# VideoVerses/VideoTuna-dev

Measured on AMD Instinct MI355X. Metric: finetune samples/sec, CogVideoX-2B T2V LoRA 49x480x720 bf16, higher is better.
Workload: dtype bf16; 1 GPU; CogVideoX-2B T2V LoRA finetune 49x480x720 (configs[1]): latents [4,13,16,60,90], text [4,226,4096], r=4 LoRA on to_q/k/v/out, 4 samples per optimizer step as in the YAML (batch_size 2 x accumulate_grad_batches 2), run as 1 micro-batch(es) of 4; mode=lora, model=CogVideoX-2B, micro_batch=4, accumulate_grad_batches=1, global_batch=4, seq_len=17776, layers=30, parallelism=dp1, recompute=none (107 GB of block activations kept in HBM), weights=seeded random init (no checkpoints offline), text=pre-encoded prompt embeddings (synthetic), latents=pre-encoded latents (synthetic)

## Files before the change

include/vt355.h:

```cpp
#ifndef VT355_H
#define VT355_H
#ifdef __cplusplus
extern "C" {
#endif

#define VT_OK 0
#define VT_ERR_BAD_SHAPE (-1)
#define VT_ERR_BAD_ALIGN (-2)
#define VT_ERR_LAUNCH (-3)
#define VT_ERR_UNSUPPORTED (-4)

int vt_version(void);
const char* vt_arch(void);
const char* vt_error_string(int code);

#define VT_EPI_BIAS 0
#define VT_EPI_BIAS_GELU 1
#define VT_EPI_GATED_RES 2
#define VT_EPI_DGELU 3

int vt_gemm_bf16(const void* A, int lda, const void* W, int ldw, void* C, int ldc,
                 int M, int N, int K, const void* bias, int epilogue, int out_fp32,
                 const void* R, int ldr, int r_mod,
                 const float* gate_txt, const float* gate_vid, int gate_bstride, int S, int St,
                 void* C2, int ldc2, const void* U, int ldu, void* stream);
int vt_gemm_set_tile(int mode);
int vt_gemm_bf16_kernel(int M, int N, int K);
int vt_conv_set_tile(int mode);

int vt_gemm_nt_bf16(const void* A, int lda, const void* B, int ldb, float* C, int ldc, int M, int P, int Q,
                    float alpha, int accumulate, void* stream);
int vt_gemm_nt_bf16_unpad(const void* A, int lda, const void* B, int ldb, float* C, int ldc, int M, int P, int Q,
                          float alpha, int accumulate, int row_group, int row_keep, int col_group, int col_keep, void* stream);

int vt_group_colsum(const void* X, int ldx, const void* Y, int ldy, const float* mean, const float* rstd,
                    float* out1, float* out2, long long M, int D, int S, int St, int grouped,
                    long long o_bstride, long long o_segstride, void* stream);

int vt_qk_ln_param_grads(const float* dq_hat, int lddq, const void* dk_hat, int lddk, const void* qkv, int ld,
                         const float* mean, const float* rstd, float* out_2x2x64, long long M, int H,
                         const float* rope_cos, const float* rope_sin, int S, int St, void* stream);
int vt_ln_param_combine(const float* G1, const float* G2, int G, int D, const void* gamma, const void* beta,
                        const float* scale_txt, const float* scale_vid, int bstride, float* dgamma, float* dbeta,
                        float* dshift_txt, float* dshift_vid, float* dscale_txt, float* dscale_vid, int dbstride,
                        int grouped, void* stream);
int vt_small_linear_bwd(const float* dy, int ldy, const void* x, int ldx, const void* W, float* dW, float* db,
                        float* dx, int lddx, int Bn, int N, int K, void* stream);
int vt_silu_bwd(const float* dy, const void* x, float* dx, long long n, void* stream);

int vt_attn_fwd_hd64(const void* q, const void* k, const void* v, void* o, float* lse2,
                     int B, int H, int S,
                     long long q_rs, long long k_rs, long long v_rs, long long o_rs,
                     long long q_bs, long long k_bs, long long v_bs, long long o_bs,
                     float softmax_scale, int q_prescaled, void* stream);

int vt_attn_fwd_bias_hd64(const void* q, const void* k, const void* v, const float* bias_t, void* o, float* lse2,
                          int B, int H, int S,
                          long long q_rs, long long k_rs, long long v_rs, long long o_rs,
                          long long q_bs, long long k_bs, long long v_bs, long long o_bs,
                          float softmax_scale, void* stream);
int vt_gemm_splitk_f32(const void* A, int lda, const void* W, int ldw, float* C, int ldc, int M, int N, int K, int splits, void* stream);
int vt_residual_cast_bf16(const float* acc, long long lda, const void* R, long long ldr, void* out, long long ldo, long long M, int N,
                          void* stream);
long long vt_groupnorm_ws_bytes(int N, int C);
int vt_groupnorm_silu_cl(const void* x, long long ldx, const void* gamma, const void* beta, void* y, long long ldy,
                         int N, long long P, int C, int G, float eps, int silu, float* ws, long long ws_bytes, void* stream);
int vt_causal_conv3d_cl(const void* x, long long ldx, const void* wk, const void* bias, const void* res, long long ldr,
                        void* y, long long ldy, int N, int T, int H, int W, int Cin, int Cout, void* stream);
int vt_downsample_conv2d_cl(const void* x, long long ldx, const void* wk, const void* bias, void* y, long long ldy,
                            int N, int T, int H, int W, int Cin, int Cout, void* stream);
int vt_causal_conv3d_in8_cl(const void* x, const void* wk, const void* bias, void* y, long long ldy,
                            int N, int T, int H, int W, int Cout, void* stream);
int vt_temporal_pool_cl(const void* x, long long ldx, void* y, long long ldy, int N, int T, long long HW, int C, int keep_first,
                        void* stream);
int vt_rmsnorm_bf16(const void* x, long long ldx, const void* w, void* y, long long ldy, long long M, int D, float eps,
                    void* stream);
int vt_gated_gelu_bf16(const void* u, long long ldu, void* y, long long ldy, long long M, int F, void* stream);

int vt_attn_bwd_hd64(const void* q, const void* k, const void* v, const void* o, const void* dout,
                     const float* lse2, float* delta_ws, float* dq_f32, void* dk, void* dv,
                     int B, int H, int S,
                     long long q_rs, long long k_rs, long long v_rs, long long o_rs, long long do_rs,
                     long long dq_rs, long long dk_rs, long long dv_rs,
                     long long q_bs, long long k_bs, long long v_bs, long long o_bs, long long do_bs,
                     long long dq_bs, long long dk_bs, long long dv_bs,
                     float softmax_scale, int q_prescaled, void* chain_ws, long long chain_ws_bytes, void* stream);
long long vt_attn_bwd_chain_ws_bytes(int B, int H, int S);
int vt_attn_bwd_set_chain(int chain_len, int slots);

int vt_ln_modulate_fwd(const void* x, int ldx, void* y, int ldy, const void* gamma, const void* beta,
                       const float* shift_txt, const float* scale_txt, const float* shift_vid,
                       const float* scale_vid, int mod_bstride, float* mean, float* rstd,
                       int M, int D, int S, int St, float eps, void* stream);
int vt_ln_modulate_bwd(const void* dy, int lddy, const void* x, int ldx, const float* mean, const float* rstd,
                       const void* gamma, const float* scale_txt, const float* scale_vid, int mod_bstride,
                       const void* dres, int lddres, void* dx, int lddx,
                       int M, int D, int S, int St, void* stream);

int vt_qk_layernorm_fwd(const void* qkv, int ld, void* out, int ldo, const void* gq, const void* bq,
                        const void* gk, const void* bk, float* mean, float* rstd,
                        long long M, int H, float eps, float q_scale,
                        const float* rope_cos, const float* rope_sin, int S, int St, void* stream);
int vt_qk_layernorm_bwd(const float* dq_hat, int lddq, const void* dk_hat, int lddk, const void* qkv, int ld,
                        const float* mean, const float* rstd, const void* gq, const void* gk,
                        void* dqkv, int ldd, long long M, int H,
                        const float* rope_cos, const float* rope_sin, int S, int St, void* stream);

int vt_gate_mul(const void* x, int ldx, void* y, int ldy, const float* g_txt, const float* g_vid, int bstride,
                long long M, int D, int S, int St, void* stream);
int vt_silu_bf16(const void* x, void* y, long long n, void* stream);
int vt_cast_f32_bf16(const float* x, void* y, long long n, void* stream);
int vt_timestep_embedding(const long long* t, void* out, int B, int D, int flip_sin_to_cos, float freq_shift,
                          void* stream);
int vt_patchify(const void* img, void* tok, int B, int F, int C, int H, int W, int P, int ldt, void* stream);
int vt_unpatchify(const void* tok, void* img, int B, int F, int C, int H, int W, int P, int ldt, void* stream);

int vt_add_noise(const float* x0, const float* noise, const float* sqrt_ab, const float* sqrt_1mab, void* noisy,
                 long long per_sample, int B, void* stream);
int vt_diffusion_loss(const void* vpred, const void* noisy, const float* x0, const float* sqrt_ab,
                      const float* sqrt_1mab, const float* weights, float* loss, float* partials_ws,
                      void* dvpred, long long per_sample, int B, float grad_scale, void* stream);

int vt_diffusion_loss_bwd(const void* vpred, const void* noisy, const float* x0, const float* sqrt_ab,
                          const float* sqrt_1mab, const float* weights, const float* grad_out, void* dvpred,
                          long long per_sample, int B, void* stream);

int vt_adamw(float* p, const float* g, float* m, float* v, void* p_bf16, long long n, float lr, float beta1,
             float beta2, float eps, float weight_decay, int step, float grad_scale, const int* guard, void* stream);

int vt_grad_sqnorm_partials(void);
int vt_grad_sqnorm(const float* g, long long n, float* partials, int slot, void* stream);
int vt_clip_finalize(const float* partials, int nslots, float grad_scale, float max_norm, float* record, void* stream);
int vt_adamw_clip(float* p, const float* g, float* m, float* v, void* p_bf16, long long n, float lr, float beta1,
                  float beta2, float eps, float weight_decay, int step, float grad_scale, const int* guard,
                  const float* clip_coef_dev, float clip_value, void* stream);

int vt_lora_down(const void* X, int ldx, const void* A, int lda, int R, void* T, int ldt, long long M, int K,
                 int zero_cols, void* stream);
int vt_skinny_tn(const void* Big, int ldb, const void* Small, int lds_, int R, float* out, long long osp,
                 long long osr, float alpha, long long M, int P, float* workspace, void* stream);
long long vt_skinny_tn_workspace_bytes(int P);
int vt_lora_up_add(void* dX, int ldx, const void* dT, int ldt, const void* A, int lda, int R, long long M, int K,
                   void* stream);
int vt_lora_pack_b(const float* Bcat, void* Wext, int ldw, int n_adapters, int d_out, int r, float scale, void* stream);
int vt_lora_pack_bt(const float* Bcat, void* WText, int ldwt, int n_adapters, int d_out, int r, float scale, void* stream);

int vt_lora_down_wide(const void* X, int ldx, const void* A, int lda, int n_adapters, int r, int rp, int ext, void* T, int ldt,
                      long long M, int K, void* stream);
int vt_lora_tn_wide(const void* Big, int ldb, const void* Small, int lds_, int R, float* out, long long osp, long long osr,
                    float alpha, long long M, int P, void* stream);
int vt_lora_up_add_wide(void* dX, int ldx, const void* dT, int ldt, const void* A, int lda, int n_adapters, int r, int rp,
                        long long M, int K, void* stream);
int vt_lora_pack_b_wide(const float* Bcat, void* Wext, int ldw, int n_adapters, int d_out, int r, int rp, int ext, float scale,
                        void* stream);
int vt_lora_pack_bt_wide(const float* Bcat, void* WText, int ldwt, int n_adapters, int d_out, int r, int rp, int ext, float scale,
                         void* stream);

int vt_lora_down_drop(const void* X, int ldx, const void* A, int lda, int R, int n_adapters, void* T, int ldt, long long M, int K,
                      int zero_cols, float p, unsigned long long seed, int site0, void* stream);
int vt_skinny_tn_drop(const void* Big, int ldb, const void* Small, int lds_, int R, int n_adapters, float* out, long long osp,
                      long long osr, float alpha, long long M, int P, float* workspace, float p, unsigned long long seed, int site0,
                      void* stream);
int vt_lora_up_add_drop(void* dX, int ldx, const void* dT, int ldt, const void* A, int lda, int R, int n_adapters, long long M, int K,
                        float p, unsigned long long seed, int site0, void* stream);
int vt_lora_down_wide_drop_fits(int n_adapters, int rp);
int vt_lora_down_wide_drop(const void* X, int ldx, const void* A, int lda, int n_adapters, int r, int rp, int ext, void* T, int ldt,
                           long long M, int K, float p, unsigned long long seed, int site0, void* stream);
int vt_lora_tn_wide_drop(const void* Big, int ldb, const void* Small, int lds_, int R, float* out, long long osp, long long osr,
                         float alpha, long long M, int P, float p, unsigned long long seed, int site, void* stream);
int vt_lora_up_add_wide_drop(void* dX, int ldx, const void* dT, int ldt, const void* A, int lda, int n_adapters, int r, int rp,
                             long long M, int K, float p, unsigned long long seed, int site0, void* stream);


int vt_conv_cl(const void* x, long long ldx, const void* wk, const void* bias, const float* sbias, int sbias_ld,
               const void* res, long long ldr, void* y, long long ldy,
               int N, int T, int H, int W, int Cin, int Cout, int KT, int KH, int KW, int pt, int ph, int pw, int stride, void* stream);
int vt_conv_dw_cl(const void* dy, long long lddy, const void* x, long long ldx, float* dw,
                  int N, int T, int H, int W, int Cin, int Cout, int KT, int KH, int KW, int pt, int ph, int pw, int stride,
                  int accumulate, void* stream);
int vt_conv_dw_bias_cl(const void* dy, long long lddy, const void* x, long long ldx, float* dw, float* dbias,
                       int N, int T, int H, int W, int Cin, int Cout, int KT, int KH, int KW, int pt, int ph, int pw, int stride,
                       int accumulate, void* stream);
int vt_transpose_bf16(const void* src, long long src_ld, long long src_boff, void* dst, long long dst_ld, long long dst_boff, int rows, int cols,
                      int nb, void* stream);
int vt_transpose_multi_bf16(const void* table, int njobs, long long total_blocks, void* stream);
int vt_conv_desc_extents(long long ldx, long long lddy, int N, int T, int H, int W, int Cin, int Cout, int KH, int KW, int ph, int pw,
                         int stride, long long* fwd_x_bytes, long long* dw_x_bytes, long long* dw_dy_bytes);
int vt_groupnorm_silu_bwd_cl(const void* dy, long long lddy, const void* x, long long ldx, const void* gamma,
                             const float* ws_fwd, float* ws_bwd, long long ws_bytes, void* dx, long long lddx,
                             float* dgamma, float* dbeta, int N, long long P, int C, int G, int silu, int accumulate, void* stream);
int vt_geglu_fwd(const void* h, long long ldh, void* y, long long ldy, long long M, int F, void* stream);
int vt_geglu_bwd(const void* dy, long long lddy, const void* h, long long ldh, void* dh, long long lddh, long long M, int F, void* stream);
int vt_add_rows_bf16(const void* a, long long lda, const void* b, long long ldb, void* out, long long ldo, long long M, int C, void* stream);
int vt_dropout_bf16(const void* x, long long ldx, void* y, long long ldy, long long M, int C, float p, unsigned long long seed,
                    unsigned long long offset, void* mask_out, void* stream);
int vt_row_map_bf16(const void* src, long long lds, void* out, long long ldo, int mode, long long nb, int d1, int d2, int C,
                    int accumulate, void* stream);
int vt_q_sample(const float* x0, const float* noise, const float* sqrt_ab, const float* sqrt_1mab, const float* scale, void* xt,
                long long per_sample, int B, void* stream);
int vt_mse_loss(const void* pred, const float* target, float* loss, void* dpred, long long total, float grad_scale, void* stream);

int vt_attn_small_fwd(const void* q, const void* k, const void* v, void* o, float* lse2, int NB, int H, int Sq, int Sk,
                      long long q_rs, long long q_bs, long long k_rs, long long k_bs, long long v_rs, long long v_bs,
                      long long o_rs, long long o_bs, float softmax_scale, int mask_block, void* stream);
int vt_attn_small_bwd(const void* q, const void* k, const void* v, const void* o, const void* dout, const float* lse2,
                      void* dq, void* dk, void* dv, float* dk32, float* dv32, int NB, int H, int Sq, int Sk,
                      long long q_rs, long long q_bs, long long k_rs, long long k_bs, long long v_rs, long long v_bs,
                      long long o_rs, long long o_bs, long long do_rs, long long do_bs, long long dq_rs, long long dq_bs,
                      long long dk_rs, long long dv_rs, float softmax_scale, int mask_block, void* stream);

long long vt_attn_dual_ws_floats(int B, int H, int Sq, int rows_per_frame, int Sa, int Sb);
int vt_attn_dual_fwd(const void* q, const void* k, const void* v, const void* k_ip, const void* v_ip, void* o, float* lse2,
                     int B, int H, int Sq, int rows_per_frame, int Sa, int Sb,
                     long long q_rs, long long q_bs, long long k_rs, long long k_bs, long long v_rs, long long v_bs,
                     long long kip_rs, long long kip_bs, long long vip_rs, long long vip_bs, long long o_rs, long long o_bs,
                     float softmax_scale, float img_scale, void* stream);
int vt_attn_dual_bwd(const void* q, const void* k, const void* v, const void* k_ip, const void* v_ip, const void* dout,
                     const float* lse2, void* dq, float* dk32, float* dv32, float* dkip32, float* dvip32, float* ws,
                     long long ws_floats, int B, int H, int Sq, int rows_per_frame, int Sa, int Sb,
                     long long q_rs, long long q_bs, long long k_rs, long long k_bs, long long v_rs, long long v_bs,
                     long long kip_rs, long long kip_bs, long long vip_rs, long long vip_bs, long long do_rs, long long do_bs,
                     long long dq_rs, long long dq_bs, float softmax_scale, float img_scale, void* stream);

int vt_attn_gen_fwd(const void* q, const void* k, const void* v, void* o, float* lse2, const int* kv_len, int head_dim, int hstride,
                    int NB, int H, int Sq, int Sk, long long q_rs, long long q_bs, long long k_rs, long long k_bs, long long v_rs,
                    long long v_bs, long long o_rs, long long o_bs, float softmax_scale, int mask_block, void* stream);
int vt_attn_gen_bwd(const void* q, const void* k, const void* v, const void* o, const void* dout, const float* lse2, const int* kv_len,
                    void* dq, void* dk, void* dv, float* dk32, float* dv32, int head_dim, int hstride, int NB, int H, int Sq, int Sk,
                    long long q_rs, long long q_bs, long long k_rs, long long k_bs, long long v_rs, long long v_bs,
                    long long o_rs, long long o_bs, long long do_rs, long long do_bs, long long dq_rs, long long dq_bs,
                    long long dk_rs, long long dv_rs, float softmax_scale, int mask_block, void* stream);

int vt_opensora_loss(const float* out, const float* x0, const float* noise, const double* coef, double* loss3, float* dout,
                     long long per_channel, int C, int B, float grad_scale, void* stream);

int vt_gemm_fp8(const void* A, int lda, const void* W, int ldw, void* C, int ldc, int M, int N, int K, const void* bias,
                const float* scale_a, const float* scale_w, void* stream);
int vt_quantize_fp8(const void* x, long long ldx, void* y, long long ldy, long long M, int K, float* scale, unsigned int* ws,
                    int given_scale, void* stream);

int vt_gemm_mxfp8(const void* A, int lda, const void* W, int ldw, void* C, int ldc, int M, int N, int K, const void* bias,
                  const float* scale_a, const float* scale_w, int epilogue, const void* residual, int ldr,
                  const float* gate_txt, const float* gate_vid, int gate_bstride, int S, int St, void* pre_act_out, int ldc2,
                  const void* At, int ldat, const void* Wt, int ldwt, int Kt, void* Cq, int ldcq, const float* scale_out,
                  unsigned int* amax, void* stream);
int vt_cast_fp8_scaled(const void* x, long long ldx, void* y, long long ldy, void* cp, long long ldcp, long long M, int K, int L,
                       int Lj, int off, const float* scale, unsigned int* amax, void* stream);
int vt_ln_modulate_fwd_fp8(const void* x, int ldx, void* y, int ldy, const void* gamma, const void* beta,
                           const float* shift_txt, const float* scale_txt, const float* shift_vid,
                           const float* scale_vid, int mod_bstride, float* mean, float* rstd,
// ... 34 lines not shown
```

videotuna-dev_amd/_lib.py:

```python
import ctypes as C
import os

_HERE = os.path.dirname(os.path.abspath(__file__))
_LIB = None


class VtError(RuntimeError):
    pass


def lib_path() -> str:
    return os.environ.get("VT355_LIB") or os.path.join(_HERE, "libvt355.so")


_vp, _i, _ll, _f, _fp = C.c_void_p, C.c_int, C.c_longlong, C.c_float, C.c_void_p
PROTOTYPES = {
    "vt_version": [],
    "vt_arch": [],
    "vt_error_string": [_i],
    "vt_gemm_bf16": [_vp, _i, _vp, _i, _vp, _i, _i, _i, _i, _vp, _i, _i, _vp, _i, _i, _fp, _fp, _i, _i, _i,
                     _vp, _i, _vp, _i, _vp],
    "vt_gemm_set_tile": [_i],
    "vt_gemm_bf16_kernel": [_i, _i, _i],
    "vt_conv_set_tile": [_i],
    "vt_transpose_bf16": [_vp, _ll, _ll, _vp, _ll, _ll, _i, _i, _i, _vp],
    "vt_transpose_multi_bf16": [_vp, _i, _ll, _vp],
    "vt_gemm_nt_bf16": [_vp, _i, _vp, _i, _fp, _i, _i, _i, _i, _f, _i, _vp],
    "vt_gemm_nt_bf16_unpad": [_vp, _i, _vp, _i, _fp, _i, _i, _i, _i, _f, _i, _i, _i, _i, _i, _vp],
    "vt_group_colsum": [_vp, _i, _vp, _i, _fp, _fp, _fp, _fp, _ll, _i, _i, _i, _i, _ll, _ll, _vp],
    "vt_qk_ln_param_grads": [_fp, _i, _vp, _i, _vp, _i, _fp, _fp, _fp, _ll, _i, _fp, _fp, _i, _i, _vp],
    "vt_ln_param_combine": [_fp, _fp, _i, _i, _vp, _vp, _fp, _fp, _i, _fp, _fp, _fp, _fp, _fp, _fp, _i, _i, _vp],
    "vt_small_linear_bwd": [_fp, _i, _vp, _i, _vp, _fp, _fp, _fp, _i, _i, _i, _i, _vp],
    "vt_silu_bwd": [_fp, _vp, _fp, _ll, _vp],
    "vt_attn_fwd_hd64": [_vp, _vp, _vp, _vp, _fp, _i, _i, _i, _ll, _ll, _ll, _ll, _ll, _ll, _ll, _ll, _f, _i, _vp],
    "vt_attn_fwd_bias_hd64": [_vp, _vp, _vp, _fp, _vp, _fp, _i, _i, _i, _ll, _ll, _ll, _ll, _ll, _ll, _ll, _ll, _f, _vp],
    "vt_gemm_splitk_f32": [_vp, _i, _vp, _i, _fp, _i, _i, _i, _i, _i, _vp],
    "vt_residual_cast_bf16": [_fp, _ll, _vp, _ll, _vp, _ll, _ll, _i, _vp],
    "vt_groupnorm_ws_bytes": [_i, _i],
    "vt_groupnorm_silu_cl": [_vp, _ll, _vp, _vp, _vp, _ll, _i, _ll, _i, _i, _f, _i, _fp, _ll, _vp],
    "vt_causal_conv3d_cl": [_vp, _ll, _vp, _vp, _vp, _ll, _vp, _ll, _i, _i, _i, _i, _i, _i, _vp],
    "vt_causal_conv3d_in8_cl": [_vp, _vp, _vp, _vp, _ll, _i, _i, _i, _i, _i, _vp],
    "vt_downsample_conv2d_cl": [_vp, _ll, _vp, _vp, _vp, _ll, _i, _i, _i, _i, _i, _i, _vp],
    "vt_temporal_pool_cl": [_vp, _ll, _vp, _ll, _i, _i, _ll, _i, _i, _vp],
    "vt_rmsnorm_bf16": [_vp, _ll, _vp, _vp, _ll, _ll, _i, _f, _vp],
    "vt_gated_gelu_bf16": [_vp, _ll, _vp, _ll, _ll, _i, _vp],
    "vt_attn_bwd_hd64": [_vp, _vp, _vp, _vp, _vp, _fp, _fp, _fp, _vp, _vp, _i, _i, _i,
                         _ll, _ll, _ll, _ll, _ll, _ll, _ll, _ll, _ll, _ll, _ll, _ll, _ll, _ll, _ll, _ll, _f, _i, _vp, _ll, _vp],
    "vt_attn_bwd_chain_ws_bytes": [_i, _i, _i],
    "vt_attn_bwd_set_chain": [_i, _i],
    "vt_ln_modulate_fwd": [_vp, _i, _vp, _i, _vp, _vp, _fp, _fp, _fp, _fp, _i, _fp, _fp, _i, _i, _i, _i, _f, _vp],
    "vt_ln_modulate_bwd": [_vp, _i, _vp, _i, _fp, _fp, _vp, _fp, _fp, _i, _vp, _i, _vp, _i, _i, _i, _i, _i, _vp],
    "vt_qk_layernorm_fwd": [_vp, _i, _vp, _i, _vp, _vp, _vp, _vp, _fp, _fp, _ll, _i, _f, _f, _fp, _fp, _i, _i, _vp],
    "vt_qk_layernorm_bwd": [_fp, _i, _vp, _i, _vp, _i, _fp, _fp, _vp, _vp, _vp, _i, _ll, _i, _fp, _fp, _i, _i, _vp],
    "vt_gate_mul": [_vp, _i, _vp, _i, _fp, _fp, _i, _ll, _i, _i, _i, _vp],
    "vt_silu_bf16": [_vp, _vp, _ll, _vp],
    "vt_cast_f32_bf16": [_fp, _vp, _ll, _vp],
    "vt_timestep_embedding": [_vp, _vp, _i, _i, _i, _f, _vp],
    "vt_patchify": [_vp, _vp, _i, _i, _i, _i, _i, _i, _i, _vp],
    "vt_unpatchify": [_vp, _vp, _i, _i, _i, _i, _i, _i, _i, _vp],
    "vt_add_noise": [_fp, _fp, _fp, _fp, _vp, _ll, _i, _vp],
    "vt_diffusion_loss": [_vp, _vp, _fp, _fp, _fp, _fp, _fp, _fp, _vp, _ll, _i, _f, _vp],
    "vt_diffusion_loss_bwd": [_vp, _vp, _fp, _fp, _fp, _fp, _fp, _vp, _ll, _i, _vp],
    "vt_adamw": [_fp, _fp, _fp, _fp, _vp, _ll, _f, _f, _f, _f, _f, _i, _f, _vp, _vp],
    "vt_grad_sqnorm_partials": [],
    "vt_grad_sqnorm": [_fp, _ll, _fp, _i, _vp],
    "vt_clip_finalize": [_fp, _i, _f, _f, _fp, _vp],
    "vt_adamw_clip": [_fp, _fp, _fp, _fp, _vp, _ll, _f, _f, _f, _f, _f, _i, _f, _vp, _fp, _f, _vp],
    "vt_lora_down": [_vp, _i, _vp, _i, _i, _vp, _i, _ll, _i, _i, _vp],
    "vt_skinny_tn": [_vp, _i, _vp, _i, _i, _fp, _ll, _ll, _f, _ll, _i, _fp, _vp],
    "vt_skinny_tn_workspace_bytes": [_i],
    "vt_lora_up_add": [_vp, _i, _vp, _i, _vp, _i, _i, _ll, _i, _vp],
    "vt_lora_pack_b": [_fp, _vp, _i, _i, _i, _i, _f, _vp],
    "vt_lora_pack_bt": [_fp, _vp, _i, _i, _i, _i, _f, _vp],
    "vt_lora_down_wide": [_vp, _i, _vp, _i, _i, _i, _i, _i, _vp, _i, _ll, _i, _vp],
    "vt_lora_tn_wide": [_vp, _i, _vp, _i, _i, _fp, _ll, _ll, _f, _ll, _i, _vp],
    "vt_lora_up_add_wide": [_vp, _i, _vp, _i, _vp, _i, _i, _i, _i, _ll, _i, _vp],
    "vt_lora_pack_b_wide": [_fp, _vp, _i, _i, _i, _i, _i, _i, _f, _vp],
    "vt_lora_pack_bt_wide": [_fp, _vp, _i, _i, _i, _i, _i, _i, _f, _vp],
    "vt_lora_down_drop": [_vp, _i, _vp, _i, _i, _i, _vp, _i, _ll, _i, _i, _f, C.c_ulonglong, _i, _vp],
    "vt_skinny_tn_drop": [_vp, _i, _vp, _i, _i, _i, _fp, _ll, _ll, _f, _ll, _i, _fp, _f, C.c_ulonglong, _i, _vp],
    "vt_lora_up_add_drop": [_vp, _i, _vp, _i, _vp, _i, _i, _i, _ll, _i, _f, C.c_ulonglong, _i, _vp],
    "vt_lora_down_wide_drop_fits": [_i, _i],
    "vt_lora_down_wide_drop": [_vp, _i, _vp, _i, _i, _i, _i, _i, _vp, _i, _ll, _i, _f, C.c_ulonglong, _i, _vp],
    "vt_lora_tn_wide_drop": [_vp, _i, _vp, _i, _i, _fp, _ll, _ll, _f, _ll, _i, _f, C.c_ulonglong, _i, _vp],
    "vt_lora_up_add_wide_drop": [_vp, _i, _vp, _i, _vp, _i, _i, _i, _i, _ll, _i, _f, C.c_ulonglong, _i, _vp],
    "vt_conv_cl": [_vp, _ll, _vp, _vp, _fp, _i, _vp, _ll, _vp, _ll] + [_i] * 13 + [_vp],
    "vt_conv_dw_cl": [_vp, _ll, _vp, _ll, _fp] + [_i] * 13 + [_i, _vp],
    "vt_conv_dw_bias_cl": [_vp, _ll, _vp, _ll, _fp, _fp] + [_i] * 13 + [_i, _vp],
    "vt_conv_desc_extents": [_ll, _ll] + [_i] * 11 + [C.POINTER(C.c_longlong)] * 3,
    "vt_groupnorm_silu_bwd_cl": [_vp, _ll, _vp, _ll, _vp, _fp, _fp, _ll, _vp, _ll, _fp, _fp, _i, _ll, _i, _i, _i, _i, _vp],
    "vt_geglu_fwd": [_vp, _ll, _vp, _ll, _ll, _i, _vp],
    "vt_geglu_bwd": [_vp, _ll, _vp, _ll, _vp, _ll, _ll, _i, _vp],
    "vt_add_rows_bf16": [_vp, _ll, _vp, _ll, _vp, _ll, _ll, _i, _vp],
    "vt_dropout_bf16": [_vp, _ll, _vp, _ll, _ll, _i, _f, C.c_ulonglong, C.c_ulonglong, _vp, _vp],
    "vt_row_map_bf16": [_vp, _ll, _vp, _ll, _i, _ll, _i, _i, _i, _i, _vp],
    "vt_q_sample": [_fp, _fp, _fp, _fp, _fp, _vp, _ll, _i, _vp],
    "vt_mse_loss": [_vp, _fp, _fp, _vp, _ll, _f, _vp],
    "vt_attn_small_fwd": [_vp, _vp, _vp, _vp, _fp, _i, _i, _i, _i] + [_ll] * 8 + [_f, _i, _vp],
    "vt_qk_rmsnorm_rope128_fwd": [_vp, _ll, _vp, _ll, _vp, _vp, _fp, _fp, _fp, _ll, _i, _i, _i, _i, _i, _f, _vp],
    "vt_qk_rmsnorm_rope128_bwd": [_vp, _ll, _vp, _ll, _vp, _ll, _vp, _vp, _fp, _fp, _fp, _fp, _fp, _ll, _i, _i, _i, _i, _i, _vp],
    "vt_attn128_fwd": [_vp, _vp, _vp, _vp, _fp, _vp, _i, _i, _i] + [_ll] * 8 + [_f, _vp],
    "vt_attn128_bwd": [_vp, _vp, _vp, _vp, _vp, _fp, _vp, _fp, _fp, _vp, _vp, _vp, _i, _i, _i] + [_ll] * 18 + [_f, _vp],
    "vt_gemm_fp8": [_vp, _i, _vp, _i, _vp, _i, _i, _i, _i, _vp, _fp, _fp, _vp],
    "vt_quantize_fp8": [_vp, _ll, _vp, _ll, _ll, _i, _fp, _vp, _i, _vp],
    "vt_gemm_mxfp8": [_vp, _i, _vp, _i, _vp, _i, _i, _i, _i, _vp, _fp, _fp, _i, _vp, _i, _fp, _fp, _i, _i, _i, _vp, _i,
                      _vp, _i, _vp, _i, _i, _vp, _i, _fp, _vp, _vp],
    "vt_cast_fp8_scaled": [_vp, _ll, _vp, _ll, _vp, _ll, _ll, _i, _i, _i, _i, _fp, _vp, _vp],
    "vt_ln_modulate_fwd_fp8": [_vp, _i, _vp, _i, _vp, _vp, _fp, _fp, _fp, _fp, _i, _fp, _fp, _i, _i, _i, _i, _f, _vp, _i, _fp, _vp, _vp],
    "vt_fp8_scale_update": [_vp, _fp, _fp, _i, _i, _vp],
    "vt_gemm_mxfp8_dx": [_vp, _i, _i, _vp, _i, _vp, _i, _i, _i, _i, _fp, _fp, _i, _vp, _i, _vp, _i, _vp, _i, _vp, _i, _i,
                         _vp, _i, _i, _fp, _vp, _vp],
    "vt_cast_fp8_fmt": [_vp, _ll, _vp, _ll, _vp, _ll, _ll, _i, _i, _i, _i, _i, _fp, _vp, _vp],
    "vt_gate_mul_fp8": [_vp, _i, _vp, _i, _fp, _fp, _i, _ll, _i, _i, _i, _vp, _i, _i, _fp, _vp, _vp],
    "vt_fp8_scale_update_fmax": [_vp, _fp, _fp, _i, _i, _f, _vp],
    "vt_opensora_loss": [_fp, _fp, _fp, _vp, _vp, _fp, _ll, _i, _i, _f, _vp],
    "vt_attn_gen_fwd": [_vp, _vp, _vp, _vp, _fp, _vp, _i, _i, _i, _i, _i, _i] + [_ll] * 8 + [_f, _i, _vp],
    "vt_attn_gen_bwd": [_vp, _vp, _vp, _vp, _vp, _fp, _vp, _vp, _vp, _vp, _fp, _fp, _i, _i, _i, _i, _i, _i] + [_ll] * 14 + [_f, _i, _vp],
    "vt_attn_small_bwd": [_vp, _vp, _vp, _vp, _vp, _fp, _vp, _vp, _vp, _fp, _fp, _i, _i, _i, _i] + [_ll] * 14 + [_f, _i, _vp],
    "vt_attn_dual_ws_floats": [_i] * 6,
    "vt_attn_dual_fwd": [_vp] * 6 + [_fp] + [_i] * 6 + [_ll] * 12 + [_f, _f, _vp],
    "vt_attn_dual_bwd": [_vp] * 6 + [_fp, _vp] + [_fp] * 5 + [_ll] + [_i] * 6 + [_ll] * 14 + [_f, _f, _vp],
}
_RESTYPE = {"vt_arch": C.c_char_p, "vt_error_string": C.c_char_p, "vt_skinny_tn_workspace_bytes": C.c_longlong,
             "vt_attn_bwd_chain_ws_bytes": C.c_longlong, "vt_groupnorm_ws_bytes": C.c_longlong,
             "vt_attn_dual_ws_floats": C.c_longlong}


def load_library():
    global _LIB
    if _LIB is not None:
        return _LIB
    import torch
    path = lib_path()
    if not os.path.exists(path):
        raise VtError(f"{path} not found: build it with `python -c 'import __graft_entry__ as g; g.build()'` "
                      f"(videotuna-dev_amd/csrc/build.sh). There is no CPU / eager fallback.")
    lib = C.CDLL(path)
    for name, args in PROTOTYPES.items():
        fn = getattr(lib, name)
        fn.argtypes = args
        fn.restype = _RESTYPE.get(name, C.c_int)
    _LIB = lib
    return lib


def check(code: int, what: str):
    if code != 0:
        lib = load_library()
        raise VtError(f"{what} failed: {lib.vt_error_string(code).decode()} (code {code})")
```

videotuna-dev_amd/csrc/attn_bwd.hip:

```cpp
#include "common.h"
#include <cstdlib>

#ifndef VT_SUFFIX
#define VT_SUFFIX
#endif
#ifndef VT_PIPE
#define VT_PIPE 1
#endif
#ifndef VT_DRAIN
#define VT_DRAIN 0
#endif
#ifndef VT_DQSHIFT
#define VT_DQSHIFT 0
#endif
#ifndef VT_STATMFMA
#define VT_STATMFMA 0
#endif
#ifndef VT_W8
#define VT_W8 1
#endif
#define BWD_THREADS (VT_W8 ? 512 : 256)
#ifndef VT_DQ16
#define VT_DQ16 0
#endif
#ifndef VT_CHAIN
#define VT_CHAIN 1
#endif
#ifndef VT_ATOM_AUX
#define VT_ATOM_AUX 0
#endif
#ifndef VT_DQPRIO
#define VT_DQPRIO 0
#endif
#ifndef VT_ABL
#define VT_ABL 0
#endif
#ifndef VT_PF
#define VT_PF 1
#endif
#define FENCE() __builtin_amdgcn_sched_barrier(0)
#ifndef DQ_RING
#define DQ_RING 2
#endif
#ifndef VT_DQ2
#define VT_DQ2 0
#endif
#ifndef VT_DMA
#define VT_DMA (VT_PF && VT_W8 && !VT_DQ16)
#endif
#ifndef VT_M16
#define VT_M16 (VT_DMA && !VT_STAMP && !VT_STATMFMA && !PF_R0 && !VT_DMA_LATE && !VT_ABL)
#endif
#ifndef VT_DS4
#define VT_DS4 (VT_M16 && !VT_DQM16)
#endif
#ifndef VT_DQM16
#define VT_DQM16 0
#endif
#ifndef VT_DMA_LATE
#define VT_DMA_LATE 0
#endif
#ifndef PF_TRN
#define PF_TRN 4
#endif
#ifndef PF_ROWN
#define PF_ROWN 2
#endif
#ifndef PF_R0
#define PF_R0 0
#endif
#ifndef VT_STAMP
#define VT_STAMP 0
#endif
#ifndef VT_CLK
#define VT_CLK 0
#endif
#define VT_CAT_(a, b) a##b
#define VT_CAT(a, b) VT_CAT_(a, b)
#define BWD_KERNEL VT_CAT(attn_bwd_hd64_kernel, VT_SUFFIX)
#define BWD_BODY VT_CAT(attn_bwd_body, VT_SUFFIX)
#define DELTA_KERNEL VT_CAT(attn_bwd_delta_kernel, VT_SUFFIX)
#define BWD_ENTRY VT_CAT(vt_attn_bwd_hd64, VT_SUFFIX)

struct AttnBwdParams {
    const bf16_t* q;
    const bf16_t* k;
    const bf16_t* v;
    const bf16_t* dout;
    const float* lse2;
    const float* delta;
    float* dq;
    bf16_t* dk;
    bf16_t* dv;
    int S, H, B;
    long long q_rs, k_rs, v_rs, do_rs, dq_rs, dk_rs, dv_rs;
    long long q_bs, k_bs, v_bs, do_bs, dq_bs, dk_bs, dv_bs;
    float scale, scale_log2;
    int chain_len;
    int* chain_ctr;
    int* chain_flags;
    int* chain_xcc;
    float* chain_tiles;
};

#define KIMG 0
#define DSIMG 32768
#define QTILE 98304
#define LSEOFF 131072
#define STATF 132096
#ifndef BWD_LDS_PAD
#define BWD_LDS_PAD 0
#endif
#define BWD_LDS (132096 + (VT_STATMFMA ? 8192 : (VT_STAMP ? 1024 : BWD_LDS_PAD)))
#if VT_STAMP
#ifndef STAMP_SLOT
#define STAMP_SLOT 40
#endif
#define STAMP_STEP 150
__device__ unsigned VT_CAT(vt_bwd_stamps, VT_SUFFIX)[256];
#define STAMP(i, dep) do { if (rec) { unsigned long long t_; asm volatile("s_memtime %0\n\ts_waitcnt lgkmcnt(0)" : "=s"(t_), "+v"(dep) :: "memory"); \
                                      if (lane == 0) ((unsigned*)(smem + 132096))[w * 16 + (i)] = (unsigned)t_; } } while (0)
#else
#define STAMP(i, dep)
#endif
#define CH_STAGE_BYTES 16384
#ifndef CH_R
#define CH_R 4
#endif
#ifndef CH_HYST
#define CH_HYST 1
#endif
#ifndef CH_SPIN_LIMIT
#define CH_SPIN_LIMIT (1 << 19)
#endif
#define CH_AUX 17

typedef __attribute__((ext_vector_type(8))) short short8v;
typedef int i32x4w __attribute__((ext_vector_type(4)));

__device__ __forceinline__ int swz_f(int row) {
    return (((row >> 1) & 1) << 2) | (((row >> 3) & 1) << 1) | ((row >> 2) & 1);
}
__device__ __forceinline__ int swz4(int row) { return (((row >> 1) & 1) << 3) | (((row >> 3) & 1) << 2) | (((row >> 2) & 1) << 1) | (row & 1); }
__device__ __forceinline__ int swz_off(int row, int chunk) { return row * 128 + ((chunk ^ swz_f(row)) << 4); }

__device__ __forceinline__ bf16x8 tr_pair(const char* p0, const char* p1) {
    short4v lo = __builtin_amdgcn_ds_read_tr16_b64_v4i16((short4v __attribute__((address_space(3)))*)(p0));
    short4v hi = __builtin_amdgcn_ds_read_tr16_b64_v4i16((short4v __attribute__((address_space(3)))*)(p1));
    short8v v8 = {lo[0], lo[1], lo[2], lo[3], hi[0], hi[1], hi[2], hi[3]};
    return __builtin_bit_cast(bf16x8, v8);
}

#if VT_W8
template <bool RAGGED, bool PRESCALED, int ROLE>
__device__ __forceinline__ void BWD_BODY(const AttnBwdParams& p, char* smem, char* stage, const int id, const int slot,
                                         const int cons_end, const int base, const bool l2_prev, const bool l2_next,
                                         bool& dead) {
    constexpr bool has_prod = (ROLE & 1) != 0, has_cons = (ROLE & 2) != 0;
    const int tid = threadIdx.x, lane = tid & 63;
    const int w = __builtin_amdgcn_readfirstlane(tid >> 6);
    const int r = lane & 31, h = lane >> 5, g = lane >> 4, ql = (lane & 15) >> 2, pl = lane & 3;
    const int nkb = (p.S + 255) / 256;
    const int kblk = id % nkb, bh = id / nkb;
    const int head = bh % p.H, b = bh / p.H;
    const int key0 = kblk * 256;

    const bf16_t* qb = p.q + (size_t)b * p.q_bs + head * 64;
    const bf16_t* kb_ = p.k + (size_t)b * p.k_bs + head * 64;
    const bf16_t* vb = p.v + (size_t)b * p.v_bs + head * 64;
    const bf16_t* dob = p.dout + (size_t)b * p.do_bs + head * 64;
    __amdgpu_buffer_rsrc_t rq = make_rsrc(qb, (unsigned)((long long)(p.S - 1) * p.q_rs * 2 + 128));
    __amdgpu_buffer_rsrc_t rk = make_rsrc(kb_, (unsigned)((long long)(p.S - 1) * p.k_rs * 2 + 128));
    __amdgpu_buffer_rsrc_t rv = make_rsrc(vb, (unsigned)((long long)(p.S - 1) * p.v_rs * 2 + 128));
    __amdgpu_buffer_rsrc_t rdo = make_rsrc(dob, (unsigned)((long long)(p.S - 1) * p.do_rs * 2 + 128));
    __amdgpu_buffer_rsrc_t rdq = make_rsrc(p.dq + (size_t)b * p.dq_bs + head * 64, (unsigned)((long long)(p.S - 1) * p.dq_rs * 4 + 256));
    const float* lse_b = p.lse2 + (size_t)bh * p.S;
    const float* dl_b = p.delta + (size_t)bh * p.S;

#pragma unroll
    for (int j = 0; j < 4; ++j) {
        const int i = tid + 512 * j;
        const int key = i >> 3, c = i & 7;
        u32x4 v = __builtin_bit_cast(u32x4, __builtin_amdgcn_raw_buffer_load_b128(rk, (int)((key0 + key) * p.k_rs * 2) + c * 16, 0, 0));
        *(u32x4*)(smem + KIMG + swz_off(key, c)) = v;
    }
#if VT_M16
    const int c15 = lane & 15;
    bf16x8 kf16[2][2], vf16[2][2];
    float kmask16[2];
#pragma unroll
    for (int kt = 0; kt < 2; ++kt) {
        const int key = key0 + 32 * w + 16 * kt + c15;
#pragma unroll
        for (int s = 0; s < 2; ++s) {
            kf16[kt][s] = __builtin_bit_cast(bf16x8, __builtin_amdgcn_raw_buffer_load_b128(rk, (int)(key * p.k_rs * 2) + (32 * s + 8 * g) * 2, 0, 0));
            vf16[kt][s] = __builtin_bit_cast(bf16x8, __builtin_amdgcn_raw_buffer_load_b128(rv, (int)(key * p.v_rs * 2) + (32 * s + 8 * g) * 2, 0, 0));
        }
        kmask16[kt] = (RAGGED && key >= p.S) ? -1.0e30f : 0.f;
    }
#else
    bf16x8 kf[4], vf[4];
    {
        const int key = key0 + 32 * w + r;
#pragma unroll
        for (int s = 0; s < 4; ++s) {
            kf[s] = __builtin_bit_cast(bf16x8, __builtin_amdgcn_raw_buffer_load_b128(rk, (int)(key * p.k_rs * 2) + (16 * s + 8 * h) * 2, 0, 0));
            vf[s] = __builtin_bit_cast(bf16x8, __builtin_amdgcn_raw_buffer_load_b128(rv, (int)(key * p.v_rs * 2) + (16 * s + 8 * h) * 2, 0, 0));
        }
    }
    const float kmask = (RAGGED && (key0 + 32 * w + r) >= p.S) ? -1.0e30f : 0.f;
#endif

#if VT_M16
    int rowrd16[2];
#pragma unroll
    for (int s_ = 0; s_ < 2; ++s_) rowrd16[s_] = c15 * 128 + (((4 * s_ + g) ^ (c15 & 6)) << 4);
    int trA16[4];
#pragma unroll
    for (int dt = 0; dt < 4; ++dt) trA16[dt] = (4 * g + ql) * 128 + (((2 * dt + (pl >> 1)) ^ ((4 * g + ql) & 6)) << 4) + (pl & 1) * 8;
#else
    int rowrd[4];
#pragma unroll
    for (int s = 0; s < 4; ++s) rowrd[s] = r * 128 + (((2 * s + h) ^ swz_f(r)) << 4);
    int trA[2][2];
#pragma unroll
    for (int dt = 0; dt < 2; ++dt)
#pragma unroll
        for (int sec = 0; sec < 2; ++sec) {
            const int fx = ((ql >> 1) << 2) | (sec << 1) | h;
            trA[dt][sec] = (4 * h + ql + 8 * sec) * 128 + (((4 * dt + 2 * (g & 1) + (pl >> 1)) ^ fx) << 4) + (pl & 1) * 8;
        }
#endif
#if VT_DQ16
    const int qt = w >> 1, dh = w & 1;
    int trq16[2], trk16[2][2];
// ... 1330 lines not shown
            for (int i = 0; i < 16; ++i) asm volatile("" ::"v"(dq_acc[i]));
#else
#pragma unroll
            for (int i = 0; i < 16; ++i)
                __builtin_amdgcn_raw_ptr_buffer_atomic_fadd_f32(dq_acc[i] * p.scale, rdq, dq_voff,
                                                                soff + ((i & 3) + 8 * (i >> 2)) * dq_rowb, 0);
#endif
        }
    }
#endif
    const float dk_mul = PRESCALED ? 0.6931471805599453f : p.scale;
#pragma unroll
    for (int kb = 0; kb < 2; ++kb) {
        const int key = key0 + 64 * w + 32 * kb + r;
        if (key < p.S) {
            bf16_t* dkp = p.dk + (size_t)b * p.dk_bs + (size_t)key * p.dk_rs + head * 64;
            bf16_t* dvp = p.dv + (size_t)b * p.dv_bs + (size_t)key * p.dv_rs + head * 64;
#pragma unroll
            for (int dt = 0; dt < 2; ++dt)
#pragma unroll
                for (int gg = 0; gg < 4; ++gg) {
                    u32x2 a, c;
                    a[0] = pack2(dk_acc[kb][dt][4 * gg + 0] * dk_mul, dk_acc[kb][dt][4 * gg + 1] * dk_mul);
                    a[1] = pack2(dk_acc[kb][dt][4 * gg + 2] * dk_mul, dk_acc[kb][dt][4 * gg + 3] * dk_mul);
                    c[0] = pack2(dv_acc[kb][dt][4 * gg + 0], dv_acc[kb][dt][4 * gg + 1]);
                    c[1] = pack2(dv_acc[kb][dt][4 * gg + 2], dv_acc[kb][dt][4 * gg + 3]);
                    *(u32x2*)(dkp + 32 * dt + 8 * gg + 4 * h) = a;
                    *(u32x2*)(dvp + 32 * dt + 8 * gg + 4 * h) = c;
                }
        }
    }
}

#endif

#if VT_CLK
__device__ unsigned VT_CAT(vt_bwd_clk, VT_SUFFIX)[4];
extern "C" int VT_CAT(vt_attn_bwd_clk, VT_SUFFIX)(unsigned* host_out) {
    return hipMemcpyFromSymbol(host_out, HIP_SYMBOL(VT_CAT(vt_bwd_clk, VT_SUFFIX)), 4 * sizeof(unsigned)) == hipSuccess ? VT_OK : VT_ERR_LAUNCH;
}
#endif
template <bool PRESCALED>
__global__ __launch_bounds__(BWD_THREADS, 1) void BWD_KERNEL(AttnBwdParams p) {
    __shared__ __attribute__((aligned(16))) char smem[BWD_LDS];
    __shared__ __attribute__((aligned(16))) char stage[CH_STAGE_BYTES];
    const int nkb = (p.S + 255) / 256;
    const int nitems = nkb * p.H * p.B, nsteps = (p.S + 63) / 64;
    const int L = p.chain_len;
    const int spx = gridDim.x >> 3;
    const int slot = (int)(blockIdx.x & 7) * spx + (int)(blockIdx.x >> 3);
    bool dead = false;
    int cons_end = 0;
    int gen = 0;
    bool l2_prev = false, l2_next = false;
#if VT_CHAIN
    if (L > 1) {
        int xcc;
        asm volatile("s_getreg_b32 %0, hwreg(HW_REG_XCC_ID)" : "=s"(xcc));
        xcc = (xcc & 15) + 1;
        __amdgpu_buffer_rsrc_t rx = make_rsrc(p.chain_xcc, (unsigned)gridDim.x * 4u);
        if (threadIdx.x == 0) __builtin_amdgcn_raw_buffer_store_b32((unsigned)xcc, rx, slot * 4, 0, CH_AUX);
        const int j = slot % spx;
        auto peer = [&](int s2) -> int {
            int v = 0, it = 0;
            while (v == 0 && it++ < (1 << 16)) {
                v = __builtin_amdgcn_readfirstlane((int)__builtin_amdgcn_raw_buffer_load_b32(rx, s2 * 4, 0, CH_AUX));
                if (v == 0) __builtin_amdgcn_s_sleep(8);
            }
            return v;
        };
        if ((j % L) != 0) {
            l2_prev = peer(slot - 1) == xcc;
            if (threadIdx.x == 0) atomicAdd(p.chain_ctr + (l2_prev ? 11 : 12), 1);
        }
        if ((j % L) != L - 1 && j != spx - 1 && slot + 1 < (int)gridDim.x) l2_next = peer(slot + 1) == xcc;
    }
#endif
    for (int item = slot; item < nitems; item += gridDim.x, ++gen) {
        const int kblk = item % nkb;
        bool has_prod = false, has_cons = false;
#if VT_CHAIN
        if (L > 1) {
            const int j = slot % spx;
            has_prod = (j % L) != 0 && kblk != 0;
            has_cons = (j % L) != L - 1 && j != spx - 1 && kblk != nkb - 1 && item + 1 < nitems;
        }
#endif
        const bool ragged = (kblk + 1) * 256 > p.S;
        const int role = (has_prod ? 1 : 0) | (has_cons ? 2 : 0);
        const int base = gen * nsteps;
#define VT_BWD_CALL(R, ROLE_) BWD_BODY<R, PRESCALED, ROLE_>(p, smem, stage, item, slot, cons_end, base, l2_prev, l2_next, dead)
#if VT_CLK
        unsigned long long clk0, rt0;
        asm volatile("s_memtime %0\n\ts_memrealtime %1\n\ts_waitcnt lgkmcnt(0)" : "=s"(clk0), "=s"(rt0) :: "memory");
#endif
#if VT_CHAIN
        switch (role) {
            case 0: if (ragged) VT_BWD_CALL(true, 0); else VT_BWD_CALL(false, 0); break;
            case 1: if (ragged) VT_BWD_CALL(true, 1); else VT_BWD_CALL(false, 1); break;
            case 2: VT_BWD_CALL(false, 2); break;
            default: VT_BWD_CALL(false, 3); break;
        }
#else
        if (ragged) VT_BWD_CALL(true, 0); else VT_BWD_CALL(false, 0);
#endif
#undef VT_BWD_CALL
#if VT_CLK
        {
            unsigned long long clk1, rt1;
            asm volatile("s_memtime %0\n\ts_memrealtime %1\n\ts_waitcnt lgkmcnt(0)" : "=s"(clk1), "=s"(rt1) :: "memory");
            if (blockIdx.x == 40 && gen == 3 && threadIdx.x == 0) {
                VT_CAT(vt_bwd_clk, VT_SUFFIX)[0] = (unsigned)(clk1 - clk0);
                VT_CAT(vt_bwd_clk, VT_SUFFIX)[1] = (unsigned)(rt1 - rt0);
            }
        }
#endif
        if (has_cons) cons_end = (gen + 1) * nsteps;
        __syncthreads();
    }
}

__global__ __launch_bounds__(256) void DELTA_KERNEL(const bf16_t* o, const bf16_t* dout, float* delta,
                                                            int B, int H, int S, long long o_rs, long long do_rs,
                                                            long long o_bs, long long do_bs) {
    const long long gid = (long long)blockIdx.x * 256 + threadIdx.x;
    const long long row = gid >> 3;
    const int sub = (int)(gid & 7);
    const long long total = (long long)B * S * H;
    float acc = 0.f;
    long long bs = 0; int hh = 0;
    if (row < total) {
        hh = (int)(row % H);
        bs = row / H;
        const int s = (int)(bs % S);
        const int b = (int)(bs / S);
        u32x4 a = *(const u32x4*)(o + (size_t)b * o_bs + (size_t)s * o_rs + hh * 64 + sub * 8);
        u32x4 c = *(const u32x4*)(dout + (size_t)b * do_bs + (size_t)s * do_rs + hh * 64 + sub * 8);
        float fa[8], fc[8];
        unpack8(a, fa);
        unpack8(c, fc);
#pragma unroll
        for (int i = 0; i < 8; ++i) acc += fa[i] * fc[i];
    }
    acc += __shfl_xor(acc, 1, 64);
    acc += __shfl_xor(acc, 2, 64);
    acc += __shfl_xor(acc, 4, 64);
    if (row < total && sub == 0) {
        const int s = (int)(bs % S);
        const int b = (int)(bs / S);
        delta[((size_t)b * H + hh) * S + s] = acc;
    }
}

static long long bwd_chain_xcc_off(long long slots) { return 256 + slots * 64; }
static long long bwd_chain_tiles_off(long long slots) { return (256 + slots * 68 + 4095) & ~4095LL; }
static long long bwd_chain_ws_bytes(long long slots) { return bwd_chain_tiles_off(slots) + slots * (long long)(CH_R * 16384); }
static int g_bwd_slots = 0;
static int g_bwd_chain = -1;
static void bwd_chain_init() {
    if (g_bwd_chain >= 0) return;
    int L = 3;
    if (const char* e = getenv("VT_BWD_CHAIN")) L = atoi(e);
    int dev = 0, cus = 0;
    if (hipGetDevice(&dev) != hipSuccess || hipDeviceGetAttribute(&cus, hipDeviceAttributeMultiprocessorCount, dev) != hipSuccess) cus = 0;
    g_bwd_slots = cus / 8 * 8;
    if (g_bwd_slots < 8) g_bwd_slots = 8;
    g_bwd_chain = L < 1 ? 1 : L;
}
static int bwd_chain_len() { bwd_chain_init(); return g_bwd_chain; }
extern "C" int VT_CAT(vt_attn_bwd_set_chain, VT_SUFFIX)(int chain_len, int slots) {
    g_bwd_chain = -1;
    bwd_chain_init();
    if (chain_len > 0) g_bwd_chain = chain_len;
    if (slots > 0) {
        if ((slots % 8) || slots > g_bwd_slots) return VT_ERR_BAD_SHAPE;
        g_bwd_slots = slots;
    }
    return VT_OK;
}

extern "C" int BWD_ENTRY(const void* q, const void* k, const void* v, const void* o, const void* dout,
                                const float* lse2, float* delta_ws, float* dq_f32, void* dk, void* dv,
                                int B, int H, int S,
                                long long q_rs, long long k_rs, long long v_rs, long long o_rs, long long do_rs,
                                long long dq_rs, long long dk_rs, long long dv_rs,
                                long long q_bs, long long k_bs, long long v_bs, long long o_bs, long long do_bs,
                                long long dq_bs, long long dk_bs, long long dv_bs,
                                float softmax_scale, int q_prescaled, void* chain_ws, long long chain_ws_bytes,
                                void* stream) {
    if (B <= 0 || H <= 0 || S <= 0) return VT_ERR_BAD_SHAPE;
    if ((long long)S * dq_rs * 4 >= 0x7fffffffLL) return VT_ERR_BAD_SHAPE;
    if ((q_rs % 8) || (k_rs % 8) || (v_rs % 8) || (o_rs % 8) || (do_rs % 8) || (dk_rs % 4) || (dv_rs % 4)) return VT_ERR_BAD_SHAPE;
    if ((q_bs % 8) || (k_bs % 8) || (v_bs % 8) || (o_bs % 8) || (do_bs % 8) || (dk_bs % 4) || (dv_bs % 4)) return VT_ERR_BAD_SHAPE;
    if ((((uintptr_t)q) | ((uintptr_t)k) | ((uintptr_t)v) | ((uintptr_t)o) | ((uintptr_t)dout)) & 15) return VT_ERR_BAD_ALIGN;
    if ((((uintptr_t)dk) | ((uintptr_t)dv)) & 7) return VT_ERR_BAD_ALIGN;
    const long long lim = 0x7fffffffLL;
    if ((long long)S * q_rs * 2 >= lim || (long long)S * k_rs * 2 >= lim || (long long)S * v_rs * 2 >= lim ||
        (long long)S * do_rs * 2 >= lim) return VT_ERR_BAD_SHAPE;
    hipStream_t st = (hipStream_t)stream;
    {
        const long long total = (long long)B * S * H * 8;
        const int blocks = (int)((total + 255) / 256);
        hipLaunchKernelGGL(DELTA_KERNEL, dim3(blocks), dim3(256), 0, st, (const bf16_t*)o, (const bf16_t*)dout,
                           delta_ws, B, H, S, o_rs, do_rs, o_bs, do_bs);
    }
    AttnBwdParams p;
    p.q = (const bf16_t*)q; p.k = (const bf16_t*)k; p.v = (const bf16_t*)v; p.dout = (const bf16_t*)dout;
    p.lse2 = lse2; p.delta = delta_ws; p.dq = dq_f32; p.dk = (bf16_t*)dk; p.dv = (bf16_t*)dv;
    p.S = S; p.H = H; p.B = B;
    p.q_rs = q_rs; p.k_rs = k_rs; p.v_rs = v_rs; p.do_rs = do_rs; p.dq_rs = dq_rs; p.dk_rs = dk_rs; p.dv_rs = dv_rs;
    p.q_bs = q_bs; p.k_bs = k_bs; p.v_bs = v_bs; p.do_bs = do_bs; p.dq_bs = dq_bs; p.dk_bs = dk_bs; p.dv_bs = dv_bs;
    p.scale = softmax_scale; p.scale_log2 = softmax_scale * 1.4426950408889634f;
    const int nkb = (S + 255) / 256;
    const long long nwg = (long long)nkb * H * B;
    if (nwg > 0x3fffffLL) return VT_ERR_BAD_SHAPE;
    p.chain_len = 1; p.chain_ctr = nullptr; p.chain_flags = nullptr; p.chain_xcc = nullptr; p.chain_tiles = nullptr;
    int L = bwd_chain_len();
    const long long pgrid = nwg < g_bwd_slots ? (nwg + 7) / 8 * 8 : g_bwd_slots;
    const long long grid = pgrid;
    if (L > pgrid / 8) L = (int)(pgrid / 8);
    if (L > nkb) L = nkb;
    if (chain_ws != nullptr && chain_ws_bytes >= 64 && !(((uintptr_t)chain_ws) & 255)) {
        char* ws = (char*)chain_ws;
        const bool on = L > 1 && chain_ws_bytes >= bwd_chain_ws_bytes(g_bwd_slots);
        if (hipMemsetAsync(ws, 0, 64, st) != hipSuccess) return VT_ERR_LAUNCH;
        if (on && hipMemsetAsync(ws + 256, 0, (size_t)bwd_chain_tiles_off(g_bwd_slots) - 256, st) != hipSuccess) return VT_ERR_LAUNCH;
        if (on) {
            p.chain_len = L;
            p.chain_ctr = (int*)ws;
            p.chain_flags = (int*)(ws + 256);
            p.chain_xcc = (int*)(ws + bwd_chain_xcc_off(g_bwd_slots));
            p.chain_tiles = (float*)(ws + bwd_chain_tiles_off(g_bwd_slots));
        }
    }
    if (q_prescaled) hipLaunchKernelGGL(BWD_KERNEL<true>, dim3((unsigned)grid), dim3(BWD_THREADS), 0, st, p);
    else hipLaunchKernelGGL(BWD_KERNEL<false>, dim3((unsigned)grid), dim3(BWD_THREADS), 0, st, p);
    return hipGetLastError() == hipSuccess ? VT_OK : VT_ERR_LAUNCH;
}

#if VT_STAMP
extern "C" int VT_CAT(vt_attn_bwd_stamps, VT_SUFFIX)(unsigned* host_out) {
    return hipMemcpyFromSymbol(host_out, HIP_SYMBOL(VT_CAT(vt_bwd_stamps, VT_SUFFIX)), 256 * sizeof(unsigned)) == hipSuccess ? VT_OK : VT_ERR_LAUNCH;
}
#endif
extern "C" long long VT_CAT(vt_attn_bwd_chain_ws_bytes, VT_SUFFIX)(int B, int H, int S) {
    if (B <= 0 || H <= 0 || S <= 0 || bwd_chain_len() <= 1) return 0;
    return bwd_chain_ws_bytes(g_bwd_slots);
}
```

videotuna-dev_amd/csrc/common.h:

```cpp
#pragma once
#include <hip/hip_runtime.h>
#include <stdint.h>

typedef __bf16 bf16_t;
typedef __attribute__((ext_vector_type(8))) __bf16 bf16x8;
typedef __attribute__((ext_vector_type(4))) __bf16 bf16x4;
typedef __attribute__((ext_vector_type(2))) __bf16 bf16x2;
typedef __attribute__((ext_vector_type(4))) short short4v;
typedef __attribute__((ext_vector_type(4))) float f32x4;
typedef __attribute__((ext_vector_type(16))) float f32x16;
typedef __attribute__((ext_vector_type(4))) int i32x4;
typedef __attribute__((ext_vector_type(2))) int i32x2;
typedef __attribute__((ext_vector_type(4))) unsigned int u32x4;
typedef __attribute__((ext_vector_type(2))) unsigned int u32x2;

#define VT_OK 0
#define VT_ERR_BAD_SHAPE (-1)
#define VT_ERR_BAD_ALIGN (-2)
#define VT_ERR_LAUNCH (-3)
#define VT_ERR_UNSUPPORTED (-4)

#define WAVE 64

__device__ __forceinline__ float bf16_bits_to_f32(unsigned short b) {
    return __uint_as_float(((unsigned int)b) << 16);
}
__device__ __forceinline__ float bf2f(bf16_t x) { return (float)x; }
__device__ __forceinline__ bf16_t f2bf(float x) { return (bf16_t)x; }

__device__ __forceinline__ void unpack8(const u32x4& v, float* f) {
#pragma unroll
    for (int i = 0; i < 4; ++i) {
        f[2 * i] = __uint_as_float(v[i] << 16);
        f[2 * i + 1] = __uint_as_float(v[i] & 0xffff0000u);
    }
}
__device__ __forceinline__ unsigned int pack2(float lo, float hi) {
    bf16x2 p;
    p[0] = (bf16_t)lo;
    p[1] = (bf16_t)hi;
    return __builtin_bit_cast(unsigned int, p);
}
__device__ __forceinline__ u32x4 pack8(const float* f) {
    u32x4 v;
#pragma unroll
    for (int i = 0; i < 4; ++i) v[i] = pack2(f[2 * i], f[2 * i + 1]);
    return v;
}

__device__ __forceinline__ float wave_sum(float v) {
#pragma unroll
    for (int o = 32; o > 0; o >>= 1) v += __shfl_xor(v, o, 64);
    return v;
}
__device__ __forceinline__ float wave_max(float v) {
#pragma unroll
    for (int o = 32; o > 0; o >>= 1) v = fmaxf(v, __shfl_xor(v, o, 64));
    return v;
}

__device__ __forceinline__ void amax_publish(unsigned int* slot, float v) {
    const unsigned int b = __float_as_uint(v);
#ifdef VT_AMAX_ALWAYS_ATOMIC
    atomicMax(slot, b);
#else
    if (b > __hip_atomic_load(slot, __ATOMIC_RELAXED, __HIP_MEMORY_SCOPE_AGENT)) atomicMax(slot, b);
#endif
}

__device__ __forceinline__ float gelu_sigmoid_f(float x, float x2) {
    const float c0 = 2.0f * 1.4426950408889634f * 0.7978845608028654f, c1 = c0 * 0.044715f;
    const float w = x * __builtin_fmaf(c1, x2, c0);
    return 1.0f - __builtin_amdgcn_rcpf(__builtin_amdgcn_exp2f(w) + 1.0f);
}
__device__ __forceinline__ float gelu_tanh_f(float x) { return x * gelu_sigmoid_f(x, x * x); }
__device__ __forceinline__ float gelu_tanh_grad_f(float x) {
    const float k0 = 0.7978845608028654f, k1 = 0.044715f;
    const float x2 = x * x;
    const float sg = gelu_sigmoid_f(x, x2);
    const float du2 = __builtin_fmaf(6.0f * k0 * k1, x2, 2.0f * k0);
    return __builtin_fmaf(x * du2, sg * (1.0f - sg), sg);
}
__device__ __forceinline__ float silu_f(float x) { return x / (1.0f + __expf(-x)); }

__device__ __forceinline__ __amdgpu_buffer_rsrc_t make_rsrc(const void* base, unsigned int bytes) {
    return __builtin_amdgcn_make_buffer_rsrc(const_cast<void*>(base), 0, (int)bytes, 0x00020000);
}

__device__ __forceinline__ int xcd_remap(int orig, int nwg) {
    const int nx = 8;
    int q = nwg / nx, r = nwg % nx;
    int xcd = orig % nx;
    int base = (xcd < r) ? xcd * (q + 1) : r * (q + 1) + (xcd - r) * q;
    return base + orig / nx;
}
__device__ __forceinline__ void rope_load8(const float* src, float* d) {
    f32x4 a = *(const f32x4*)src, b = *(const f32x4*)(src + 4);
#pragma unroll
    for (int j = 0; j < 4; ++j) { d[j] = a[j]; d[j + 4] = b[j]; }
}
__device__ __forceinline__ void rope_bwd8(const float* rope_cos, const float* rope_sin, int spos, int sub, float* dy) {
    float cs[8], sn[8];
    rope_load8(rope_cos + (size_t)spos * 64 + sub * 8, cs);
    rope_load8(rope_sin + (size_t)spos * 64 + sub * 8, sn);
#pragma unroll
    for (int j = 0; j < 8; j += 2) {
        const float a = dy[j], b = dy[j + 1];
        dy[j] = a * cs[j] + b * sn[j + 1];
        dy[j + 1] = b * cs[j + 1] - a * sn[j];
    }
}

__device__ __forceinline__ void philox4x32_10(unsigned c0, unsigned c1, unsigned c2, unsigned c3, unsigned k0, unsigned k1, unsigned* out) {
#pragma unroll
    for (int r = 0; r < 10; ++r) {
        const unsigned long long p0 = (unsigned long long)0xD2511F53u * c0, p1 = (unsigned long long)0xCD9E8D57u * c2;
        const unsigned n0 = (unsigned)(p1 >> 32) ^ c1 ^ k0, n1 = (unsigned)p1, n2 = (unsigned)(p0 >> 32) ^ c3 ^ k1, n3 = (unsigned)p0;
        c0 = n0; c1 = n1; c2 = n2; c3 = n3;
        k0 += 0x9E3779B9u; k1 += 0xBB67AE85u;
    }
    out[0] = c0; out[1] = c1; out[2] = c2; out[3] = c3;
}
static inline unsigned vt_keep_thresh(float p) {
    const double t = (double)p * 4294967296.0;
    return t >= 4294967295.0 ? 0xffffffffu : (unsigned)t;
}
__device__ __forceinline__ void keep_words4(unsigned long long ctr, unsigned long long seed, unsigned* rnd) {
    philox4x32_10((unsigned)ctr, (unsigned)(ctr >> 32), 0u, 0u, (unsigned)seed, (unsigned)(seed >> 32), rnd);
}
__device__ __forceinline__ u32x4 keep_mask8(u32x4 v, unsigned long long ctr, unsigned long long seed, unsigned thresh) {
    unsigned rnd[8];
    keep_words4(ctr, seed, rnd);
    keep_words4(ctr + 1, seed, rnd + 4);
#pragma unroll
    for (int i = 0; i < 4; ++i) v[i] &= (rnd[2 * i] >= thresh ? 0x0000ffffu : 0u) | (rnd[2 * i + 1] >= thresh ? 0xffff0000u : 0u);
    return v;
}
__device__ __forceinline__ unsigned long long lora_site_offset(int site) { return (unsigned long long)site << 36; }
struct LoraDrop {
    unsigned thresh;
    float inv_keep;
    unsigned long long seed;
    int site0;
    int n, r;
    long long mbase;
};
__device__ __forceinline__ LoraDrop lora_drop_arg() { return LoraDrop{}; }
__device__ __forceinline__ LoraDrop lora_drop_arg(const LoraDrop& d) { return d; }
static inline LoraDrop vt_lora_drop(float p, unsigned long long seed, int site0, int n = 0, int r = 0) {
    return LoraDrop{vt_keep_thresh(p), 1.0f / (1.0f - p), seed, site0, n, r, 0};
}
static inline int vt_lora_drop_bad(float p, int site0) { return !(p >= 0.f) || !(p < 1.f) || site0 < 0 || site0 > (1 << 20); }
```

videotuna-dev_amd/csrc/lora.hip:

```cpp
#include "common.h"
#include <cstdlib>

static int lora_drop_args_bad(int R, int n, float p, int site0) {
    return n <= 0 || n > 3 || R <= 0 || R > 16 || (R % n) || vt_lora_drop_bad(p, site0);
}

template <typename... D>
__global__ __launch_bounds__(256) void lora_down_kernel(const bf16_t* X, int ldx, const bf16_t* A, int lda, int R,
                                                       bf16_t* T, int ldt, long long M, int K, int zero_cols, D... drop) {
    constexpr bool DROP = sizeof...(D) > 0;
    const LoraDrop dr = lora_drop_arg(drop...);
    const int lane = threadIdx.x & 63, wave = threadIdx.x >> 6;
    const long long row0 = ((long long)blockIdx.x * 4 + wave) * 16;
    if (row0 >= M) return;
    const int fr = lane & 15, fq = lane >> 4;
    long long xr = row0 + fr;
    if (xr > M - 1) xr = M - 1;
    const bf16_t* xp = X + (size_t)xr * ldx + 16 * fq;
    const bool aok = fr < R;
    const bf16_t* ap = A + (size_t)(aok ? fr : 0) * lda + 16 * fq;
    const int ja = DROP ? fr / dr.r : 0;
    const unsigned long long e4 = DROP ? ((unsigned long long)xr * K + 16 * fq) >> 2 : 0;
    f32x4 acc = {0.f, 0.f, 0.f, 0.f};
    const u32x4 zero = {0u, 0u, 0u, 0u};
// ... 79 lines not shown
#pragma unroll
            for (int c = 0; c < 4; ++c) acc[c][rr] += bm[ja][c] * s[j];
        }
    }
}
template <int RR, int NA, int RPER, typename... D>
__global__ __launch_bounds__(128) void skinny_tn_kernel(const bf16_t* Big, int ldb, const bf16_t* Small, int lds_, int R,
                                                       float* out, long long osp, long long osr, float alpha,
                                                       long long M, int P, int rows_per_slice, float* ws, D... drop) {
    static_assert((NA > 0) == (sizeof...(D) > 0), "the mask needs the dropout argument");
    const LoraDrop dr = lora_drop_arg(drop...);
    __shared__ __attribute__((aligned(16))) float sm[SK_MAXROWS * RR];
    const long long m0 = (long long)blockIdx.y * rows_per_slice;
    const int p = (blockIdx.x * 128 + threadIdx.x) * 4;
    const int rows = m0 < M ? (int)((M - m0) < rows_per_slice ? (M - m0) : rows_per_slice) : 0;
    for (int i = threadIdx.x; i < rows * RR; i += 128) {
        const int mm = i / RR, rr = i - mm * RR;
        sm[i] = rr < R ? bf2f(Small[(size_t)(m0 + mm) * lds_ + rr]) : 0.f;
    }
    __syncthreads();
    const bool valid = p < P;
    float acc[4][RR];
#pragma unroll
    for (int c = 0; c < 4; ++c)
#pragma unroll
        for (int rr = 0; rr < RR; ++rr) acc[c][rr] = 0.f;
    const bf16_t* bp = Big + (size_t)m0 * ldb + (valid ? p : 0);
    const unsigned long long e40 = NA > 0 ? ((unsigned long long)(dr.mbase + m0) * P + p) >> 2 : 0, estep = (unsigned long long)(P >> 2);
    int mb = 0;
    for (; valid && mb + 16 <= rows; mb += 16) {
        u32x2 raw[16];
#pragma unroll
        for (int u = 0; u < 16; ++u) raw[u] = *(const u32x2*)(bp + (size_t)(mb + u) * ldb);
#pragma unroll
        for (int u = 0; u < 16; ++u) sk_row<RR, NA, RPER>(raw[u], sm + (mb + u) * RR, e40 + (mb + u) * estep, dr, acc);
    }
    for (; valid && mb < rows; ++mb)
        sk_row<RR, NA, RPER>(*(const u32x2*)(bp + (size_t)mb * ldb), sm + mb * RR, e40 + mb * estep, dr, acc);
    if (ws != nullptr) {
        if (!valid) return;
        float* w = ws + ((size_t)(blockIdx.y % SK_COPIES) * P + p) * RR;
#pragma unroll
        for (int c = 0; c < 4; ++c)
#pragma unroll
            for (int rr = 0; rr < RR; ++rr)
                if (rr < R) atomicAdd(w + c * RR + rr, acc[c][rr]);
    } else {
        __syncthreads();
        const int pl = threadIdx.x * 4;
        const int pb0 = blockIdx.x * 512;
#pragma unroll
        for (int c = 0; c < 4; ++c)
#pragma unroll
            for (int rr = 0; rr < RR; ++rr) sm[(pl + c) * RR + rr] = alpha * acc[c][rr];
        __syncthreads();
        if (osr == 1) {
            for (int i = threadIdx.x; i < 512 * RR; i += 128) {
                const int pp = i / RR, rr = i - pp * RR;
                if (rr < R && pb0 + pp < P) atomicAdd(out + (size_t)(pb0 + pp) * osp + rr, sm[i]);
            }
        } else {
            for (int rr = 0; rr < R; ++rr)
                for (int pp = threadIdx.x; pp < 512; pp += 128)
                    if (pb0 + pp < P) atomicAdd(out + (size_t)(pb0 + pp) * osp + (size_t)rr * osr, sm[pp * RR + rr]);
        }
    }
}
template <int RR>
__global__ __launch_bounds__(256) void skinny_reduce_kernel(const float* ws, int nslices, float* out, long long osp, long long osr,
                                                           float alpha, int P, int R) {
    const int i = blockIdx.x * 256 + threadIdx.x;
    if (i >= P * RR) return;
    const int p = i / RR, rr = i - p * RR;
    if (rr >= R) return;
    float s = 0.f;
    for (int k = 0; k < nslices; ++k) s += ws[(size_t)k * P * RR + i];
    out[(size_t)p * osp + (size_t)rr * osr] += alpha * s;
}
extern "C" long long vt_skinny_tn_workspace_bytes(int P) { return (long long)SK_COPIES * P * 16 * 4; }
#define SK_ARGS bg, ldb, smp, lds_, R, out, osp, osr, alpha, mc, P, rps, workspace
#define SK_DROP_LAUNCH(RR_, NA_, RPER_) \
    hipLaunchKernelGGL((skinny_tn_kernel<RR_, NA_, RPER_, LoraDrop>), grid, dim3(128), 0, st, SK_ARGS, drm)
static int skinny_tn_launch(const void* Big, int ldb, const void* Small, int lds_, int R, float* out, long long osp, long long osr,
                            float alpha, long long M, int P, float* workspace, int nsl, const LoraDrop* dr, void* stream) {
    if (M <= 0 || P <= 0 || (P % 4) || R <= 0 || R > 16 || (ldb % 4)) return VT_ERR_BAD_SHAPE;
    if (((uintptr_t)Big) & 7) return VT_ERR_BAD_ALIGN;
    if (workspace != nullptr && (((uintptr_t)workspace) & 15)) return VT_ERR_BAD_ALIGN;
    hipStream_t st = (hipStream_t)stream;
    const long long chunk = (long long)nsl * SK_MAXROWS;
    const int RRw = R <= 4 ? 4 : 16;
    if (workspace != nullptr && hipMemsetAsync(workspace, 0, (size_t)SK_COPIES * P * RRw * 4, st) != hipSuccess) return VT_ERR_LAUNCH;
    for (long long mbase = 0; mbase < M; mbase += chunk) {
        const long long mc = (M - mbase) < chunk ? (M - mbase) : chunk;
        const int rps = (int)((mc + nsl - 1) / nsl);
        dim3 grid((P + 511) / 512, nsl);
        const bf16_t* bg = (const bf16_t*)Big + (size_t)mbase * ldb;
        const bf16_t* smp = (const bf16_t*)Small + (size_t)mbase * lds_;
        if (dr == nullptr) {
            if (R <= 4) hipLaunchKernelGGL((skinny_tn_kernel<4, 0, 1>), grid, dim3(128), 0, st, SK_ARGS);
            else hipLaunchKernelGGL((skinny_tn_kernel<16, 0, 1>), grid, dim3(128), 0, st, SK_ARGS);
        } else {
            LoraDrop drm = *dr;
            drm.mbase = mbase;
            if (dr->n == 1) {
                if (R <= 4) SK_DROP_LAUNCH(4, 1, 16); else SK_DROP_LAUNCH(16, 1, 16);
            } else if (dr->r == 1) SK_DROP_LAUNCH(4, 3, 1);
            else if (dr->r == 2) SK_DROP_LAUNCH(16, 3, 2);
            else if (dr->r == 3) SK_DROP_LAUNCH(16, 3, 3);
            else if (dr->r == 4) SK_DROP_LAUNCH(16, 3, 4);
            else SK_DROP_LAUNCH(16, 3, 5);
        }
    }
    if (workspace != nullptr) {
        if (R <= 4) hipLaunchKernelGGL(skinny_reduce_kernel<4>, dim3((P * 4 + 255) / 256), dim3(256), 0, st, workspace, SK_COPIES, out, osp, osr, alpha, P, R);
        else hipLaunchKernelGGL(skinny_reduce_kernel<16>, dim3((P * 16 + 255) / 256), dim3(256), 0, st, workspace, SK_COPIES, out, osp, osr, alpha, P, R);
    }
    return hipGetLastError() == hipSuccess ? VT_OK : VT_ERR_LAUNCH;
}
#undef SK_DROP_LAUNCH
#undef SK_ARGS
extern "C" int vt_skinny_tn(const void* Big, int ldb, const void* Small, int lds_, int R, float* out, long long osp,
                            long long osr, float alpha, long long M, int P, float* workspace, void* stream) {
    static int slices_env = -1;
    if (slices_env < 0) { const char* e = getenv("VT_SK_SLICES"); slices_env = e ? atoi(e) : 0; }
    const int nsl = (slices_env > 0 && slices_env <= 1024) ? slices_env : SK_SLICES;
    return skinny_tn_launch(Big, ldb, Small, lds_, R, out, osp, osr, alpha, M, P, workspace, nsl, nullptr, stream);
}
extern "C" int vt_skinny_tn_drop(const void* Big, int ldb, const void* Small, int lds_, int R, int n_adapters, float* out, long long osp,
                                 long long osr, float alpha, long long M, int P, float* workspace, float p, unsigned long long seed,
                                 int site0, void* stream) {
    if (lora_drop_args_bad(R, n_adapters, p, site0) || n_adapters == 2) return VT_ERR_BAD_SHAPE;
    const LoraDrop dr = vt_lora_drop(p, seed, site0, n_adapters, R / n_adapters);
    return skinny_tn_launch(Big, ldb, Small, lds_, R, out, osp, osr, alpha * dr.inv_keep, M, P, workspace, SK_SLICES, &dr, stream);
}

template <typename... D>
__global__ __launch_bounds__(256) void lora_up_add_kernel(bf16_t* dX, int ldx, const bf16_t* dT, int ldt, const bf16_t* A, int lda,
                                                         int R, long long M, int K, D... drop) {
    constexpr bool DROP = sizeof...(D) > 0;
    const LoraDrop dr = lora_drop_arg(drop...);
    const int n = DROP ? dr.n : 1, r = DROP ? dr.r : R;
    const int nch = K >> 3;
    const long long total = M * nch;
    for (long long i = (long long)blockIdx.x * 256 + threadIdx.x; i < total; i += (long long)gridDim.x * 256) {
        const long long m = i / nch;
        const int c = (int)(i - m * nch);
        float v[8];
        unpack8(*(const u32x4*)(dX + (size_t)m * ldx + c * 8), v);
        for (int j = 0; j < n; ++j) {
            float s[8] = {0.f, 0.f, 0.f, 0.f, 0.f, 0.f, 0.f, 0.f};
            float(&acc)[8] = DROP ? s : v;
            for (int ri = j * r; ri < (j + 1) * r; ++ri) {
                const float t = bf2f(dT[(size_t)m * ldt + ri]);
                float a[8];
                unpack8(*(const u32x4*)(A + (size_t)ri * lda + c * 8), a);
#pragma unroll
                for (int q = 0; q < 8; ++q) acc[q] += t * a[q];
            }
            if constexpr (DROP) {
                unsigned rnd[8];
                const unsigned long long ctr = lora_site_offset(dr.site0 + j) + (((unsigned long long)m * K + 8 * c) >> 2);
                keep_words4(ctr, dr.seed, rnd);
                keep_words4(ctr + 1, dr.seed, rnd + 4);
#pragma unroll
                for (int q = 0; q < 8; ++q) v[q] += rnd[q] >= dr.thresh ? dr.inv_keep * s[q] : 0.f;
            }
        }
        *(u32x4*)(dX + (size_t)m * ldx + c * 8) = pack8(v);
    }
}
static int lora_up_add_launch(void* dX, int ldx, const void* dT, int ldt, const void* A, int lda, int R, long long M, int K,
                              const LoraDrop* dr, void* stream) {
    if (M <= 0 || K <= 0 || (K % 8) || R <= 0 || R > 16 || (ldx % 8) || (lda % 8)) return VT_ERR_BAD_SHAPE;
    if ((((uintptr_t)dX) | ((uintptr_t)A)) & 15) return VT_ERR_BAD_ALIGN;
    long long total = M * (K >> 3), b = (total + 255) / 256;
    const dim3 grid((unsigned)(b > 8192 ? 8192 : b));
    if (dr == nullptr)
        hipLaunchKernelGGL(lora_up_add_kernel<>, grid, dim3(256), 0, (hipStream_t)stream, (bf16_t*)dX, ldx, (const bf16_t*)dT, ldt,
                           (const bf16_t*)A, lda, R, M, K);
    else
        hipLaunchKernelGGL(lora_up_add_kernel<LoraDrop>, grid, dim3(256), 0, (hipStream_t)stream, (bf16_t*)dX, ldx, (const bf16_t*)dT, ldt,
                           (const bf16_t*)A, lda, R, M, K, *dr);
    return hipGetLastError() == hipSuccess ? VT_OK : VT_ERR_LAUNCH;
}
extern "C" int vt_lora_up_add(void* dX, int ldx, const void* dT, int ldt, const void* A, int lda, int R, long long M, int K,
                              void* stream) {
    return lora_up_add_launch(dX, ldx, dT, ldt, A, lda, R, M, K, nullptr, stream);
}
extern "C" int vt_lora_up_add_drop(void* dX, int ldx, const void* dT, int ldt, const void* A, int lda, int R, int n_adapters, long long M,
                                   int K, float p, unsigned long long seed, int site0, void* stream) {
    if (lora_drop_args_bad(R, n_adapters, p, site0)) return VT_ERR_BAD_SHAPE;
    const LoraDrop dr = vt_lora_drop(p, seed, site0, n_adapters, R / n_adapters);
    return lora_up_add_launch(dX, ldx, dT, ldt, A, lda, R, M, K, &dr, stream);
}

__global__ void lora_pack_b_kernel(const float* Bcat, bf16_t* Wext, int ldw, int n_adapters, int d_out, int r, float scale) {
    const int i = blockIdx.x * 256 + threadIdx.x;
    const int total = n_adapters * d_out * 64;
    if (i >= total) return;
    const int n = i >> 6, c = i & 63;
    const int j = n / d_out;
    float v = 0.f;
    if (c >= j * r && c < (j + 1) * r) v = scale * Bcat[(size_t)n * r + (c - j * r)];
    Wext[(size_t)n * ldw + c] = f2bf(v);
}
extern "C" int vt_lora_pack_b(const float* Bcat, void* Wext, int ldw, int n_adapters, int d_out, int r, float scale,
                              void* stream) {
    if (n_adapters <= 0 || d_out <= 0 || r <= 0 || n_adapters * r > 64) return VT_ERR_BAD_SHAPE;
    const int total = n_adapters * d_out * 64;
    hipLaunchKernelGGL(lora_pack_b_kernel, dim3((total + 255) / 256), dim3(256), 0, (hipStream_t)stream, Bcat, (bf16_t*)Wext, ldw,
                       n_adapters, d_out, r, scale);
    return hipGetLastError() == hipSuccess ? VT_OK : VT_ERR_LAUNCH;
}

__global__ void lora_pack_bt_kernel(const float* Bcat, bf16_t* WText, int ldwt, int n_adapters, int d_out, int r, float scale) {
    const int i = blockIdx.x * 256 + threadIdx.x;
    const int N = n_adapters * d_out;
    if (i >= 64 * N) return;
    const int c = i / N, n = i - c * N;
    const int j = n / d_out;
    float v = 0.f;
    if (c >= j * r && c < (j + 1) * r) v = scale * Bcat[(size_t)n * r + (c - j * r)];
    WText[(size_t)c * ldwt + n] = f2bf(v);
}
extern "C" int vt_lora_pack_bt(const float* Bcat, void* WText, int ldwt, int n_adapters, int d_out, int r, float scale,
                               void* stream) {
    if (n_adapters <= 0 || d_out <= 0 || r <= 0 || n_adapters * r > 64) return VT_ERR_BAD_SHAPE;
    const int total = n_adapters * d_out * 64;
    hipLaunchKernelGGL(lora_pack_bt_kernel, dim3((total + 255) / 256), dim3(256), 0, (hipStream_t)stream, Bcat, (bf16_t*)WText, ldwt,
                       n_adapters, d_out, r, scale);
    return hipGetLastError() == hipSuccess ? VT_OK : VT_ERR_LAUNCH;
}
```

videotuna-dev_amd/csrc/norm.hip:

```cpp
#include "common.h"

#define LN_MAXCH 8

struct LnParams {
    const bf16_t* x; int ldx;
    bf16_t* y; int ldy;
    const bf16_t* gamma; const bf16_t* beta;
    const float* shift_txt; const float* scale_txt; const float* shift_vid; const float* scale_vid;
    int mod_bstride;
    float* mean; float* rstd;
    int M, D, S, St;
    float eps;
    unsigned char* q; int ldq; const float* qscale; unsigned int* amax;
};

template <int NCH, bool Q = false>
__global__ __launch_bounds__(256) void ln_modulate_fwd_kernel(LnParams p) {
    const int lane = threadIdx.x & 63;
    const int m = blockIdx.x * 4 + (threadIdx.x >> 6);
    if (m >= p.M) return;
    const int nchunks = p.D >> 3;
    const bf16_t* xr = p.x + (size_t)m * p.ldx;
    float v[NCH][8];
    float sum = 0.f;
#pragma unroll
    for (int i = 0; i < NCH; ++i) {
        const int c = lane + 64 * i;
        if (c < nchunks) {
            u32x4 raw = *(const u32x4*)(xr + c * 8);
            unpack8(raw, v[i]);
#pragma unroll
            for (int j = 0; j < 8; ++j) sum += v[i][j];
        } else {
#pragma unroll
            for (int j = 0; j < 8; ++j) v[i][j] = 0.f;
        }
    }
    const float mean = wave_sum(sum) / (float)p.D;
    float sq = 0.f;
#pragma unroll
    for (int i = 0; i < NCH; ++i) {
        const int c = lane + 64 * i;
        if (c < nchunks) {
#pragma unroll
            for (int j = 0; j < 8; ++j) { float d = v[i][j] - mean; sq += d * d; }
        }
    }
    const float rstd = rsqrtf(wave_sum(sq) / (float)p.D + p.eps);
    if (lane == 0 && p.mean != nullptr) { p.mean[m] = mean; p.rstd[m] = rstd; }
    const float* sh = nullptr; const float* scp = nullptr;
    if (p.shift_vid != nullptr) {
        const int b = m / p.S;
        const int s = m - b * p.S;
        sh = (s < p.St ? p.shift_txt : p.shift_vid) + (size_t)b * p.mod_bstride;
        scp = (s < p.St ? p.scale_txt : p.scale_vid) + (size_t)b * p.mod_bstride;
    }
    bf16_t* yr = p.y + (size_t)m * p.ldy;
    float qmax = 0.f;
#pragma unroll
    for (int i = 0; i < NCH; ++i) {
        const int c = lane + 64 * i;
        if (c < nchunks) {
            float o[8];
            float ga[8], be[8];
            if (p.gamma != nullptr) {
                unpack8(*(const u32x4*)(p.gamma + c * 8), ga);
                unpack8(*(const u32x4*)(p.beta + c * 8), be);
            }
#pragma unroll
            for (int j = 0; j < 8; ++j) {
                float t = (v[i][j] - mean) * rstd;
                if (p.gamma != nullptr) t = t * ga[j] + be[j];
                o[j] = t;
            }
            if (sh != nullptr) {
                f32x4 s0 = *(const f32x4*)(scp + c * 8), s1 = *(const f32x4*)(scp + c * 8 + 4);
                f32x4 h0 = *(const f32x4*)(sh + c * 8), h1 = *(const f32x4*)(sh + c * 8 + 4);
#pragma unroll
                for (int j = 0; j < 4; ++j) {
                    o[j] = o[j] * (1.f + s0[j]) + h0[j];
                    o[j + 4] = o[j + 4] * (1.f + s1[j]) + h1[j];
                }
            }
            const u32x4 packed = pack8(o);
            *(u32x4*)(yr + c * 8) = packed;
            if constexpr (Q) {
                float b[8];
                unpack8(packed, b);
                const float qs = p.qscale[0];
                unsigned int w[2];
#pragma unroll
                for (int h = 0; h < 2; ++h) {
                    float t[4];
#pragma unroll
                    for (int j = 0; j < 4; ++j) {
                        qmax = fmaxf(qmax, fabsf(b[4 * h + j]));
                        t[j] = fminf(fmaxf(__fdiv_rn(b[4 * h + j], qs), -448.0f), 448.0f);
                    }
                    int r = 0;
                    r = __builtin_amdgcn_cvt_pk_fp8_f32(t[0], t[1], r, false);
                    r = __builtin_amdgcn_cvt_pk_fp8_f32(t[2], t[3], r, true);
                    w[h] = (unsigned int)r;
                }
                *(u32x2*)(p.q + (size_t)m * p.ldq + c * 8) = (u32x2){w[0], w[1]};
            }
        }
    }
    if constexpr (Q) {
        qmax = wave_max(qmax);
        if (lane == 0) amax_publish(p.amax, qmax);
    }
}

struct LnBwdParams {
    const bf16_t* dy; int lddy;
    const bf16_t* x; int ldx;
    const float* mean; const float* rstd;
    const bf16_t* gamma;
    const float* scale_txt; const float* scale_vid; int mod_bstride;
    const bf16_t* dres; int lddres;
    bf16_t* dx; int lddx;
    int M, D, S, St;
};

template <int NCH>
__global__ __launch_bounds__(256) void ln_modulate_bwd_kernel(LnBwdParams p) {
    const int lane = threadIdx.x & 63;
    const int m = blockIdx.x * 4 + (threadIdx.x >> 6);
    if (m >= p.M) return;
    const int nchunks = p.D >> 3;
    const float mean = p.mean[m], rstd = p.rstd[m];
    const float* scp = nullptr;
    if (p.scale_vid != nullptr) {
        const int b = m / p.S;
        const int s = m - b * p.S;
        scp = (s < p.St ? p.scale_txt : p.scale_vid) + (size_t)b * p.mod_bstride;
    }
    float gv[NCH][8], xh[NCH][8];
    float s1 = 0.f, s2 = 0.f;
#pragma unroll
    for (int i = 0; i < NCH; ++i) {
        const int c = lane + 64 * i;
        if (c < nchunks) {
            float dyv[8], xv[8];
            unpack8(*(const u32x4*)(p.dy + (size_t)m * p.lddy + c * 8), dyv);
            unpack8(*(const u32x4*)(p.x + (size_t)m * p.ldx + c * 8), xv);
            float ga[8];
            if (p.gamma != nullptr) unpack8(*(const u32x4*)(p.gamma + c * 8), ga);
            float sc8[8];
            if (scp != nullptr) {
                f32x4 a = *(const f32x4*)(scp + c * 8), bq = *(const f32x4*)(scp + c * 8 + 4);
#pragma unroll
                for (int j = 0; j < 4; ++j) { sc8[j] = 1.f + a[j]; sc8[j + 4] = 1.f + bq[j]; }
            }
#pragma unroll
            for (int j = 0; j < 8; ++j) {
                float gg = dyv[j];
                if (scp != nullptr) gg *= sc8[j];
                if (p.gamma != nullptr) gg *= ga[j];
                float xhat = (xv[j] - mean) * rstd;
                gv[i][j] = gg;
                xh[i][j] = xhat;
                s1 += gg;
                s2 += gg * xhat;
            }
        } else {
#pragma unroll
            for (int j = 0; j < 8; ++j) { gv[i][j] = 0.f; xh[i][j] = 0.f; }
        }
    }
    const float invD = 1.f / (float)p.D;
    const float m1 = wave_sum(s1) * invD, m2 = wave_sum(s2) * invD;
#pragma unroll
    for (int i = 0; i < NCH; ++i) {
        const int c = lane + 64 * i;
        if (c < nchunks) {
            float o[8];
#pragma unroll
            for (int j = 0; j < 8; ++j) o[j] = rstd * (gv[i][j] - m1 - xh[i][j] * m2);
            if (p.dres != nullptr) {
                float dr[8];
                unpack8(*(const u32x4*)(p.dres + (size_t)m * p.lddres + c * 8), dr);
#pragma unroll
                for (int j = 0; j < 8; ++j) o[j] += dr[j];
            }
            *(u32x4*)(p.dx + (size_t)m * p.lddx + c * 8) = pack8(o);
        }
    }
}

static int nch_for(int D) { return ((D >> 3) + 63) / 64; }

extern "C" int vt_ln_modulate_fwd(const void* x, int ldx, void* y, int ldy, const void* gamma, const void* beta,
                                  const float* shift_txt, const float* scale_txt, const float* shift_vid,
                                  const float* scale_vid, int mod_bstride, float* mean, float* rstd,
                                  int M, int D, int S, int St, float eps, void* stream) {
    if (M <= 0 || D <= 0 || (D % 8) || D > 4096 || (ldx % 8) || (ldy % 8)) return VT_ERR_BAD_SHAPE;
    if ((gamma == nullptr) != (beta == nullptr)) return VT_ERR_BAD_SHAPE;
    if (shift_vid != nullptr && (shift_txt == nullptr || scale_txt == nullptr || scale_vid == nullptr || (mod_bstride % 4)))
        return VT_ERR_BAD_SHAPE;
    if ((((uintptr_t)x) | ((uintptr_t)y)) & 15) return VT_ERR_BAD_ALIGN;
    LnParams p{(const bf16_t*)x, ldx, (bf16_t*)y, ldy, (const bf16_t*)gamma, (const bf16_t*)beta,
               shift_txt, scale_txt, shift_vid, scale_vid, mod_bstride, mean, rstd, M, D, S > 0 ? S : 1, St, eps};
    dim3 grid((M + 3) / 4), block(256);
    hipStream_t st = (hipStream_t)stream;
    const int nch = nch_for(D);
    if (nch <= 1) hipLaunchKernelGGL(ln_modulate_fwd_kernel<1>, grid, block, 0, st, p);
    else if (nch <= 4) hipLaunchKernelGGL(ln_modulate_fwd_kernel<4>, grid, block, 0, st, p);
    else hipLaunchKernelGGL(ln_modulate_fwd_kernel<8>, grid, block, 0, st, p);
    return hipGetLastError() == hipSuccess ? VT_OK : VT_ERR_LAUNCH;
}

extern "C" int vt_ln_modulate_fwd_fp8(const void* x, int ldx, void* y, int ldy, const void* gamma, const void* beta,
                                      const float* shift_txt, const float* scale_txt, const float* shift_vid,
                                      const float* scale_vid, int mod_bstride, float* mean, float* rstd,
                                      int M, int D, int S, int St, float eps, void* q, int ldq, const float* qscale, unsigned int* amax,
                                      void* stream) {
    if (M <= 0 || D <= 0 || (D % 8) || D > 4096 || (ldx % 8) || (ldy % 8) || (ldq % 8) || ldq < D) return VT_ERR_BAD_SHAPE;
    if (q == nullptr || qscale == nullptr || amax == nullptr) return VT_ERR_BAD_SHAPE;
    if ((gamma == nullptr) != (beta == nullptr)) return VT_ERR_BAD_SHAPE;
    if (shift_vid != nullptr && (shift_txt == nullptr || scale_txt == nullptr || scale_vid == nullptr || (mod_bstride % 4)))
        return VT_ERR_BAD_SHAPE;
    if ((((uintptr_t)x) | ((uintptr_t)y)) & 15 || (((uintptr_t)q) & 7)) return VT_ERR_BAD_ALIGN;
    LnParams p{(const bf16_t*)x, ldx, (bf16_t*)y, ldy, (const bf16_t*)gamma, (const bf16_t*)beta,
               shift_txt, scale_txt, shift_vid, scale_vid, mod_bstride, mean, rstd, M, D, S > 0 ? S : 1, St, eps,
               (unsigned char*)q, ldq, qscale, amax};
    dim3 grid((M + 3) / 4), block(256);
    hipStream_t st = (hipStream_t)stream;
    const int nch = nch_for(D);
    if (nch <= 1) hipLaunchKernelGGL((ln_modulate_fwd_kernel<1, true>), grid, block, 0, st, p);
    else if (nch <= 4) hipLaunchKernelGGL((ln_modulate_fwd_kernel<4, true>), grid, block, 0, st, p);
    else hipLaunchKernelGGL((ln_modulate_fwd_kernel<8, true>), grid, block, 0, st, p);
    return hipGetLastError() == hipSuccess ? VT_OK : VT_ERR_LAUNCH;
}

extern "C" int vt_ln_modulate_bwd(const void* dy, int lddy, const void* x, int ldx, const float* mean, const float* rstd,
                                  const void* gamma, const float* scale_txt, const float* scale_vid, int mod_bstride,
                                  const void* dres, int lddres, void* dx, int lddx,
                                  int M, int D, int S, int St, void* stream) {
    if (M <= 0 || D <= 0 || (D % 8) || D > 4096 || (ldx % 8) || (lddy % 8) || (lddx % 8)) return VT_ERR_BAD_SHAPE;
    if (dres != nullptr && (lddres % 8)) return VT_ERR_BAD_SHAPE;
    if (scale_vid != nullptr && (scale_txt == nullptr || (mod_bstride % 4))) return VT_ERR_BAD_SHAPE;
    if ((((uintptr_t)x) | ((uintptr_t)dy) | ((uintptr_t)dx) | ((uintptr_t)dres)) & 15) return VT_ERR_BAD_ALIGN;
    LnBwdParams p{(const bf16_t*)dy, lddy, (const bf16_t*)x, ldx, mean, rstd, (const bf16_t*)gamma,
                  scale_txt, scale_vid, mod_bstride, (const bf16_t*)dres, lddres, (bf16_t*)dx, lddx,
                  M, D, S > 0 ? S : 1, St};
    dim3 grid((M + 3) / 4), block(256);
    hipStream_t st = (hipStream_t)stream;
    const int nch = nch_for(D);
    if (nch <= 1) hipLaunchKernelGGL(ln_modulate_bwd_kernel<1>, grid, block, 0, st, p);
    else if (nch <= 4) hipLaunchKernelGGL(ln_modulate_bwd_kernel<4>, grid, block, 0, st, p);
    else hipLaunchKernelGGL(ln_modulate_bwd_kernel<8>, grid, block, 0, st, p);
    return hipGetLastError() == hipSuccess ? VT_OK : VT_ERR_LAUNCH;
}

__global__ __launch_bounds__(256) void qk_layernorm_fwd_kernel(const bf16_t* qkv, int ld, bf16_t* out, int ldo,
                                                              const bf16_t* gq, const bf16_t* bq, const bf16_t* gk,
                                                              const bf16_t* bk, float* mean, float* rstd,
                                                              long long M, int H, float eps, float q_scale,
                                                              const float* rope_cos, const float* rope_sin, int S, int St) {
    const long long gid = (long long)blockIdx.x * 256 + threadIdx.x;
    const long long grp = gid >> 3;
    const int sub = (int)(gid & 7);
    const long long total = M * 2 * H;
    const bool ok = grp < total;
    const long long m = ok ? grp / (2 * H) : 0;
    const int wh = ok ? (int)(grp % (2 * H)) : 0;
    float v[8];
    if (ok) unpack8(*(const u32x4*)(qkv + (size_t)m * ld + wh * 64 + sub * 8), v);
    else {
#pragma unroll
        for (int j = 0; j < 8; ++j) v[j] = 0.f;
    }
    float s = 0.f;
#pragma unroll
    for (int j = 0; j < 8; ++j) s += v[j];
    s += __shfl_xor(s, 1, 64); s += __shfl_xor(s, 2, 64); s += __shfl_xor(s, 4, 64);
    const float mu = s * (1.f / 64.f);
    float q = 0.f;
#pragma unroll
    for (int j = 0; j < 8; ++j) { float d = v[j] - mu; q += d * d; }
    q += __shfl_xor(q, 1, 64); q += __shfl_xor(q, 2, 64); q += __shfl_xor(q, 4, 64);
    const float rs = rsqrtf(q * (1.f / 64.f) + eps);
    if (!ok) return;
    const bool isk = wh >= H;
    float ga[8], be[8];
    unpack8(*(const u32x4*)((isk ? gk : gq) + sub * 8), ga);
    unpack8(*(const u32x4*)((isk ? bk : bq) + sub * 8), be);
    const float osc = isk ? 1.0f : q_scale;
    float o[8];
#pragma unroll
    for (int j = 0; j < 8; ++j) o[j] = (v[j] - mu) * rs * ga[j] + be[j];
    const int spos = rope_cos != nullptr ? (int)(m % S) - St : -1;
    if (spos >= 0) {
        float cs[8], sn[8];
        rope_load8(rope_cos + (size_t)spos * 64 + sub * 8, cs);
        rope_load8(rope_sin + (size_t)spos * 64 + sub * 8, sn);
#pragma unroll
        for (int j = 0; j < 8; j += 2) {
            const float a = o[j], b = o[j + 1];
            o[j] = a * cs[j] - b * sn[j];
            o[j + 1] = b * cs[j + 1] + a * sn[j + 1];
        }
    }
#pragma unroll
    for (int j = 0; j < 8; ++j) o[j] *= osc;
    *(u32x4*)(out + (size_t)m * ldo + wh * 64 + sub * 8) = pack8(o);
    if (sub == 0) { mean[m * 2 * H + wh] = mu; rstd[m * 2 * H + wh] = rs; }
}

__global__ __launch_bounds__(256) void qk_layernorm_bwd_kernel(const float* dqh, int lddq, const bf16_t* dkh, int lddk,
                                                              const bf16_t* qkv, int ld, const float* mean,
                                                              const float* rstd, const bf16_t* gq, const bf16_t* gk,
                                                              bf16_t* dqkv, int ldd, long long M, int H,
                                                              const float* rope_cos, const float* rope_sin, int S, int St) {
    const long long gid = (long long)blockIdx.x * 256 + threadIdx.x;
    const long long grp = gid >> 3;
    const int sub = (int)(gid & 7);
    const long long total = M * 2 * H;
    const bool ok = grp < total;
    const long long m = ok ? grp / (2 * H) : 0;
    const int wh = ok ? (int)(grp % (2 * H)) : 0;
    const bool isk = wh >= H;
    float g[8], xh[8];
    float mu = 0.f, rs = 0.f;
    if (ok) {
        mu = mean[m * 2 * H + wh];
        rs = rstd[m * 2 * H + wh];
        float dy[8], xv[8], ga[8];
        if (isk) {
            unpack8(*(const u32x4*)(dkh + (size_t)m * lddk + (wh - H) * 64 + sub * 8), dy);
        } else {
            const float* src = dqh + (size_t)m * lddq + wh * 64 + sub * 8;
            f32x4 a = *(const f32x4*)src, b = *(const f32x4*)(src + 4);
#pragma unroll
            for (int j = 0; j < 4; ++j) { dy[j] = a[j]; dy[j + 4] = b[j]; }
        }
        const int spos = rope_cos != nullptr ? (int)(m % S) - St : -1;
        if (spos >= 0) rope_bwd8(rope_cos, rope_sin, spos, sub, dy);
        unpack8(*(const u32x4*)(qkv + (size_t)m * ld + wh * 64 + sub * 8), xv);
        unpack8(*(const u32x4*)((isk ? gk : gq) + sub * 8), ga);
#pragma unroll
        for (int j = 0; j < 8; ++j) { g[j] = dy[j] * ga[j]; xh[j] = (xv[j] - mu) * rs; }
    } else {
#pragma unroll
        for (int j = 0; j < 8; ++j) { g[j] = 0.f; xh[j] = 0.f; }
    }
    float s1 = 0.f, s2 = 0.f;
#pragma unroll
    for (int j = 0; j < 8; ++j) { s1 += g[j]; s2 += g[j] * xh[j]; }
    s1 += __shfl_xor(s1, 1, 64); s1 += __shfl_xor(s1, 2, 64); s1 += __shfl_xor(s1, 4, 64);
    s2 += __shfl_xor(s2, 1, 64); s2 += __shfl_xor(s2, 2, 64); s2 += __shfl_xor(s2, 4, 64);
    if (!ok) return;
    const float m1 = s1 * (1.f / 64.f), m2 = s2 * (1.f / 64.f);
    float o[8];
#pragma unroll
    for (int j = 0; j < 8; ++j) o[j] = rs * (g[j] - m1 - xh[j] * m2);
    *(u32x4*)(dqkv + (size_t)m * ldd + wh * 64 + sub * 8) = pack8(o);
}

extern "C" int vt_qk_layernorm_fwd(const void* qkv, int ld, void* out, int ldo, const void* gq, const void* bq,
                                   const void* gk, const void* bk, float* mean, float* rstd,
                                   long long M, int H, float eps, float q_scale,
                                   const float* rope_cos, const float* rope_sin, int S, int St, void* stream) {
    if (M <= 0 || H <= 0 || (ld % 8) || (ldo % 8) || ld < 2 * H * 64 || ldo < 2 * H * 64) return VT_ERR_BAD_SHAPE;
    if ((rope_cos == nullptr) != (rope_sin == nullptr)) return VT_ERR_BAD_SHAPE;
    if (rope_cos != nullptr && (S <= 0 || St < 0 || St > S || (M % S))) return VT_ERR_BAD_SHAPE;
    if ((((uintptr_t)rope_cos) | ((uintptr_t)rope_sin)) & 15) return VT_ERR_BAD_ALIGN;
    if ((((uintptr_t)qkv) | ((uintptr_t)out) | ((uintptr_t)gq) | ((uintptr_t)bq) | ((uintptr_t)gk) | ((uintptr_t)bk)) & 15)
        return VT_ERR_BAD_ALIGN;
    const long long threads = M * 2 * H * 8;
    const long long blocks = (threads + 255) / 256;
    if (blocks > 0x7fffffffLL) return VT_ERR_BAD_SHAPE;
    hipLaunchKernelGGL(qk_layernorm_fwd_kernel, dim3((unsigned)blocks), dim3(256), 0, (hipStream_t)stream,
                       (const bf16_t*)qkv, ld, (bf16_t*)out, ldo, (const bf16_t*)gq, (const bf16_t*)bq,
                       (const bf16_t*)gk, (const bf16_t*)bk, mean, rstd, M, H, eps, q_scale, rope_cos, rope_sin,
                       S > 0 ? S : 1, St);
    return hipGetLastError() == hipSuccess ? VT_OK : VT_ERR_LAUNCH;
}

extern "C" int vt_qk_layernorm_bwd(const float* dq_hat, int lddq, const void* dk_hat, int lddk, const void* qkv, int ld,
                                   const float* mean, const float* rstd, const void* gq, const void* gk,
                                   void* dqkv, int ldd, long long M, int H,
                                   const float* rope_cos, const float* rope_sin, int S, int St, void* stream) {
    if (M <= 0 || H <= 0 || (ld % 8) || (ldd % 8) || (lddq % 4) || (lddk % 8)) return VT_ERR_BAD_SHAPE;
    if ((rope_cos == nullptr) != (rope_sin == nullptr)) return VT_ERR_BAD_SHAPE;
    if (rope_cos != nullptr && (S <= 0 || St < 0 || St > S || (M % S))) return VT_ERR_BAD_SHAPE;
    if ((((uintptr_t)rope_cos) | ((uintptr_t)rope_sin)) & 15) return VT_ERR_BAD_ALIGN;
    if ((((uintptr_t)qkv) | ((uintptr_t)dqkv) | ((uintptr_t)dq_hat) | ((uintptr_t)dk_hat) | ((uintptr_t)gq) | ((uintptr_t)gk)) & 15)
        return VT_ERR_BAD_ALIGN;
    const long long threads = M * 2 * H * 8;
    const long long blocks = (threads + 255) / 256;
    if (blocks > 0x7fffffffLL) return VT_ERR_BAD_SHAPE;
    hipLaunchKernelGGL(qk_layernorm_bwd_kernel, dim3((unsigned)blocks), dim3(256), 0, (hipStream_t)stream,
                       dq_hat, lddq, (const bf16_t*)dk_hat, lddk, (const bf16_t*)qkv, ld, mean, rstd,
                       (const bf16_t*)gq, (const bf16_t*)gk, (bf16_t*)dqkv, ldd, M, H, rope_cos, rope_sin, S > 0 ? S : 1, St);
    return hipGetLastError() == hipSuccess ? VT_OK : VT_ERR_LAUNCH;
}
```

videotuna-dev_amd/engine.py:

```python
from __future__ import annotations

from types import SimpleNamespace
from typing import List, Optional

import torch

from . import ops
from .ops import BF16, EPI_BIAS, EPI_BIAS_GELU, EPI_DGELU, EPI_GATED_RES

EXT = 64
Q_PRESCALE = 1.4426950408889634 / 8.0


def _lin(mod):
    base = getattr(mod, "base_layer", mod)
    return base.weight, base.bias


def _ext_widths(model):
    st = model.lora
    return (st.ext_qkv, st.ext_o) if st is not None else (EXT, EXT)


def _ext_rows(w: torch.Tensor, ext: int) -> torch.Tensor:
    out = torch.zeros(w.shape[0], w.shape[1] + ext, dtype=BF16, device=w.device)
    out[:, :w.shape[1]] = w
    return out


def _ext_t(w: torch.Tensor, ext: int) -> torch.Tensor:
    out = torch.zeros(w.shape[1] + ext, w.shape[0], dtype=BF16, device=w.device)
    out[:w.shape[1]] = w.t()
    return out


def pack(model) -> SimpleNamespace:
    ft = getattr(model, "fullft", None)
    if ft is None and any(p.requires_grad for n, p in model.named_parameters() if "lora" not in n):
        raise RuntimeError("base weights require grad but no training state exists: call vt355.fullft.enable_full_finetune(model) "
                           "for full fine-tuning, or freeze the base (requires_grad_(False)) and inject LoRA adapters")
    for n, p in model.named_parameters():
        if "lora" not in n and p.dtype != BF16:
            raise TypeError(f"parameter {n} is {p.dtype}; the MI355X engine computes in bf16 -- call .bfloat16()")
    eq, eo = _ext_widths(model)
    P = SimpleNamespace(layers=[], lora_version=-1, ft_version=-1 if ft is None else ft.version, ext=(eq, eo))
    d = model.inner_dim
    with torch.no_grad():
        for i, blk in enumerate(model.transformer_blocks):
            a = blk.attn1
            wq, bq = _lin(a.to_q); wk, bk = _lin(a.to_k); wv, bv = _lin(a.to_v); wo, bo = _lin(a.to_out[0])
            L = SimpleNamespace()
            if ft is not None:
                pre = f"transformer_blocks.{i}.attn1."
                L.w_qkv = ft.span(ft.flat_bf16, pre + "to_q.weight", pre + "to_v.weight", (3 * d, d))
                L.b_qkv = ft.span(ft.flat_bf16, pre + "to_q.bias", pre + "to_v.bias", (3 * d,))
                L.w_qkv_t = L.w_qkv.t().contiguous()
                L.w_o, L.b_o, L.w_o_t = wo, bo, wo.t().contiguous()
            else:
                wqkv = torch.cat([wq, wk, wv], 0)
                L.w_qkv = _ext_rows(wqkv, eq); L.b_qkv = torch.cat([bq, bk, bv]).contiguous(); L.w_qkv_t = _ext_t(wqkv, eq)
                L.w_o = _ext_rows(wo, eo); L.b_o = bo; L.w_o_t = _ext_t(wo, eo)
            w1, b1 = _lin(blk.ff.net[0].proj); w2, b2 = _lin(blk.ff.net[2])
            L.w1, L.b1, L.w1_t = w1, b1, w1.t().contiguous()
            L.w2, L.b2, L.w2_t = w2, b2, w2.t().contiguous()
            L.n1g, L.n1b = blk.norm1.norm.weight, blk.norm1.norm.bias
            L.n2g, L.n2b = blk.norm2.norm.weight, blk.norm2.norm.bias
            L.gq, L.bq, L.gk, L.bk = a.norm_q.weight, a.norm_q.bias, a.norm_k.weight, a.norm_k.bias
            P.layers.append(L)
        if ft is not None:
            nl = model.config.num_layers
            nmod = (12 * nl + 2) * d
            P.w_ada = ft.span(ft.flat_bf16, "transformer_blocks.0.norm1.linear.weight", "norm_out.linear.weight",
                              (nmod, model.config.time_embed_dim))
            P.b_ada = ft.span(ft.flat_bf16, "transformer_blocks.0.norm1.linear.bias", "norm_out.linear.bias", (nmod,))
        else:
            ada_w = [m.linear.weight for blk in model.transformer_blocks for m in (blk.norm1, blk.norm2)]
            ada_b = [m.linear.bias for blk in model.transformer_blocks for m in (blk.norm1, blk.norm2)]
            P.w_ada = torch.cat(ada_w + [model.norm_out.linear.weight], 0).contiguous()
            P.b_ada = torch.cat(ada_b + [model.norm_out.linear.bias], 0).contiguous()
        pw = model.patch_embed.proj.weight
        P.patch_w = pw.reshape(pw.shape[0], -1).contiguous()
        P.patch_b = model.patch_embed.proj.bias
        P.text_w, P.text_b = _lin(model.patch_embed.text_proj)
        P.t1_w, P.t1_b = _lin(model.time_embedding.linear_1)
        P.t2_w, P.t2_b = _lin(model.time_embedding.linear_2)
        P.proj_w, P.proj_b = _lin(model.proj_out)
        P.proj_w_t = P.proj_w.t().contiguous()
    return P


def packed(model) -> SimpleNamespace:
    ft = getattr(model, "fullft", None)
    if (model._packed is None or (ft is not None and model._packed.ft_version != ft.version)
            or model._packed.ext != _ext_widths(model)):
        model._packed = pack(model)
    P = model._packed
    st = model.lora
    if st is not None and P.lora_version != st.version:
        d, r, rp, eq, eo = model.inner_dim, st.r, st.rp, st.ext_qkv, st.ext_o
        for i, L in enumerate(P.layers):
            if st.wide:
                ops.lora_pack_b_wide(st.b_qkv(st.flat, i), L.w_qkv[:, d:], d + eq, 3, d, r, rp, eq, st.scaling)
                ops.lora_pack_bt_wide(st.b_qkv(st.flat, i), L.w_qkv_t[d:], 3 * d, 3, d, r, rp, eq, st.scaling)
                ops.lora_pack_b_wide(st.b_out(st.flat, i), L.w_o[:, d:], d + eo, 1, d, r, rp, eo, st.scaling)
                ops.lora_pack_bt_wide(st.b_out(st.flat, i), L.w_o_t[d:], d, 1, d, r, rp, eo, st.scaling)
                continue
            ops.lora_pack_b(st.b_qkv(st.flat, i), L.w_qkv[:, d:], d + eq, 3, d, r, st.scaling)
            ops.lora_pack_bt(st.b_qkv(st.flat, i), L.w_qkv_t[d:], 3 * d, 3, d, r, st.scaling)
            ops.lora_pack_b(st.b_out(st.flat, i), L.w_o[:, d:], d + eo, 1, d, r, st.scaling)
            ops.lora_pack_bt(st.b_out(st.flat, i), L.w_o_t[d:], d, 1, d, r, st.scaling)
        P.lora_version = st.version
    return P


def lora_dropout_seed(model):
    st = model.lora
    if st is None or not getattr(st, "p", 0.0) or not model.training:
        return None
    seed = getattr(model, "lora_dropout_seed", None)
    if seed is None:
        seed = int(torch.randint(0, 2 ** 62, (1,)).item())
    model.last_lora_dropout_seed = int(seed)
    return float(st.p), int(seed)


def _lora_proj(st, i, proj, buf):
    if proj == "qkv":
        return 3, st.a_qkv(buf, i), st.ext_qkv, 4 * i
    return 1, st.a_out(buf, i), st.ext_o, 4 * i + 3


def _narrow_calls(n, r):
    return [(0, n)] if n * r <= 16 else [(j, 1) for j in range(n)]


def _lora_down(st, i, proj, x, d, drop=None):
    n, a, ext, site = _lora_proj(st, i, proj, st.flat_bf16)
    r, rp = st.r, st.rp
    if st.wide:
        if drop is None:
            ops.lora_down_wide(x, a, n, r, rp, ext, x[:, d:], d)
        elif ops.lora_down_wide_drop_fits(n, rp):
            ops.lora_down_wide_drop(x, a, n, r, rp, ext, x[:, d:], d, *drop, site)
        else:
            for j in range(n):
                ops.lora_down_wide_drop(x, a[j * r:(j + 1) * r], 1, r, rp, rp if j < n - 1 else ext - j * rp, x[:, d + j * rp:], d,
                                        *drop, site + j)
        return
    for j, nj in _narrow_calls(n, r):
        zc = EXT - 16 - j * r if j + nj == n else 0
        if drop is None:
            ops.lora_down(x, a[j * r:(j + nj) * r], nj * r, x[:, d + j * r:], d, zero_cols=zc)
        else:
            ops.lora_down_drop(x, a[j * r:(j + nj) * r], nj * r, nj, x[:, d + j * r:], d, *drop, site + j, zero_cols=zc)
# ... 85 lines not shown
    a = SimpleNamespace(h_in=h)
    x1 = E(M, d + eq)
    a.mean1, a.rstd1 = E(M, dt=torch.float32), E(M, dt=torch.float32)
    ops.ln_modulate_fwd(h, x1, Lw.n1g, Lw.n1b, (m1.shift_txt, m1.scale_txt, m1.shift_vid, m1.scale_vid, m1.bs),
                        a.mean1, a.rstd1, d, S, St, c.norm_eps)
    if st is not None:
        _lora_down(st, i, "qkv", x1, d, drop)
    qkv = E(M, 3 * d)
    ops.gemm(x1, Lw.w_qkv, qkv, Lw.b_qkv, K=KEq)
    qkh = E(M, 2 * d)
    a.qmean, a.qrstd = E(M, 2 * H, dt=torch.float32), E(M, 2 * H, dt=torch.float32)
    ops.qk_layernorm_fwd(qkv, qkh, Lw.gq, Lw.bq, Lw.gk, Lw.bk, a.qmean, a.qrstd, H, 1e-6, q_scale=Q_PRESCALE, rope=rope)
    o = E(M, d + eo)
    lse = E(B, H, S, dt=torch.float32)
    qk3, qkv3, o3 = qkh.view(B, S, 2 * d), qkv.view(B, S, 3 * d), o.view(B, S, d + eo)
    ops.attn_fwd(qk3[:, :, :d], qk3[:, :, d:], qkv3[:, :, 2 * d:], o3[:, :, :d], lse, B, H, S, q_prescaled=True)
    if st is not None:
        _lora_down(st, i, "out", o, d, drop)
    h1 = E(M, d)
    ao = E(M, d) if (save and ft is not None) else None
    ops.gemm(o, Lw.w_o, h1, Lw.b_o, epilogue=EPI_GATED_RES, residual=h, gate_txt=m1.gate_txt, gate_vid=m1.gate_vid,
             gate_bstride=m1.bs, S=S, St=St, K=KEo, pre_act_out=ao)
    a.mean2, a.rstd2 = E(M, dt=torch.float32), E(M, dt=torch.float32)
    keep_ff = save and ft is not None
    x2 = E(M, d) if keep_ff else xg
    gact = E(M, c.ff_mult * d) if keep_ff else gbuf
    ops.ln_modulate_fwd(h1, x2, Lw.n2g, Lw.n2b, (m2.shift_txt, m2.scale_txt, m2.shift_vid, m2.scale_vid, m2.bs),
                        a.mean2, a.rstd2, d, S, St, c.norm_eps)
    u = E(M, c.ff_mult * d) if save else gbuf.new_empty(M, c.ff_mult * d)
    ops.gemm(x2, Lw.w1, gact, Lw.b1, epilogue=EPI_BIAS_GELU, pre_act_out=u)
    h2 = E(M, d)
    fo = E(M, d) if keep_ff else None
    ops.gemm(gact, Lw.w2, h2, Lw.b2, epilogue=EPI_GATED_RES, residual=h1, gate_txt=m2.gate_txt, gate_vid=m2.gate_vid,
             gate_bstride=m2.bs, S=S, St=St, pre_act_out=fo)
    if save:
        a.x1, a.qkv, a.qkh, a.o, a.lse, a.h1, a.u = x1, qkv, qkh, o, lse, h1, u
        a.x2, a.g, a.ao, a.fo = (x2, gact, ao, fo) if ft is not None else (None, None, None, None)
    return h2, a


def run_forward(model, x, text, t, save: bool, rope=None):
    c = model.config
    P = packed(model)
    st = model.lora
    d, H, L = model.inner_dim, c.num_attention_heads, c.num_layers
    B, Fr, C, Hh, Ww = x.shape
    p = c.patch_size
    Sv, St = Fr * (Hh // p) * (Ww // p), text.shape[1]
    S = St + Sv
    M = B * S
    dev = x.device
    ft = getattr(model, "fullft", None)
    E = lambda *s, dt=BF16: torch.empty(*s, dtype=dt, device=dev)

    te = c.time_embed_dim
    tsin = E(B, d); ops.timestep_embedding(t, tsin, c.flip_sin_to_cos, float(c.freq_shift))
    e1_pre = E(B, te); ops.gemm(tsin, P.t1_w, e1_pre, P.t1_b)
    e1 = E(B, te); ops.silu(e1_pre, e1)
    emb_pre = E(B, te); ops.gemm(e1, P.t2_w, emb_pre, P.t2_b)
    emb = E(B, te); ops.silu(emb_pre, emb)
    mod = E(B, P.w_ada.shape[0], dt=torch.float32); ops.gemm(emb, P.w_ada, mod, P.b_ada)

    h = E(M, d)
    patches = E(B * Sv, C * p * p); ops.patchify(x, patches, p)
    pos = model.pos_table(Fr, Hh, Ww, dev)
    pos_txt = model.patch_embed.pos_embedding[0, :St] if c.use_learned_positional_embeddings else None
    for b in range(B):
        if pos is not None:
            ops.gemm(patches[b * Sv:(b + 1) * Sv], P.patch_w, h[b * S + St:(b + 1) * S], P.patch_b,
                     epilogue=EPI_GATED_RES, residual=pos)
        else:
            ops.gemm(patches[b * Sv:(b + 1) * Sv], P.patch_w, h[b * S + St:(b + 1) * S], P.patch_b)
        if pos_txt is not None:
            ops.gemm(text[b], P.text_w, h[b * S:b * S + St], P.text_b, epilogue=EPI_GATED_RES, residual=pos_txt)
        else:
            ops.gemm(text[b], P.text_w, h[b * S:b * S + St], P.text_b)
    if rope is not None:
        rope = (rope[0], rope[1], S, St)

    dims = (B, Fr, C, Hh, Ww, S, St, Sv, M)
    scratch = SimpleNamespace(xg=E(M, d), gbuf=E(M, c.ff_mult * d))
    recompute = save and _use_recompute(model, dims)
    drop = lora_dropout_seed(model)
    saved: List[SimpleNamespace] = []
    for i in range(L):
        h2, a = block_forward(model, i, h, mod, dims, rope, save and not recompute, scratch, drop)
        if save:
            saved.append(a)
        h = h2

    mo = 2 * L * 6 * d
    f_shift, f_scale = mod[:, mo:], mod[:, mo + d:]
    y1 = E(B * Sv, d); y2 = E(B * Sv, d)
    fm1, fr1 = E(B * Sv, dt=torch.float32), E(B * Sv, dt=torch.float32)
    fm2, fr2 = E(B * Sv, dt=torch.float32), E(B * Sv, dt=torch.float32)
    for b in range(B):
        rows = slice(b * Sv, (b + 1) * Sv)
        ops.ln_modulate_fwd(h[b * S + St:(b + 1) * S], y1[rows], model.norm_final.weight, model.norm_final.bias, None,
                            fm1[rows], fr1[rows], d, Sv, 0, c.norm_eps)
    ops.ln_modulate_fwd(y1, y2, model.norm_out.norm.weight, model.norm_out.norm.bias,
                        (f_shift, f_scale, f_shift, f_scale, mod.stride(0)), fm2, fr2, d, Sv, 0, c.norm_eps)
    tok = E(B * Sv, P.proj_w.shape[0])
    ops.gemm(y2, P.proj_w, tok, P.proj_b)
    out = E(B, Fr, c.out_channels, Hh, Ww)
    ops.unpatchify(tok, out, p)
    ctx = None
    if save:
        ctx = SimpleNamespace(blocks=saved, mod=mod, h_last=h, y1=y1, fm1=fm1, fr1=fr1, fm2=fm2, fr2=fr2,
                              dims=dims, f_scale=f_scale, rope=rope, recompute=recompute, scratch=scratch if recompute else None,
                              lora_drop=drop)
        if ft is not None:
            ctx.y2, ctx.tsin, ctx.e1_pre, ctx.e1, ctx.emb_pre, ctx.se, ctx.patches, ctx.text = y2, tsin, e1_pre, e1, emb_pre, emb, patches, text
    return out, ctx


def run_backward(model, ctx, dout: torch.Tensor):
    c = model.config
    P = packed(model)
    st = model.lora
    d, H, L = model.inner_dim, c.num_attention_heads, c.num_layers
    B, Fr, C, Hh, Ww, S, St, Sv, M = ctx.dims
    p = c.patch_size
    dev = dout.device
    r, rp = st.r, st.rp
    eq, eo = st.ext_qkv, st.ext_o
    tn = ops.lora_tn_wide if st.wide else ops.skinny_tn
    E = lambda *s, dt=BF16: torch.empty(*s, dtype=dt, device=dev)
    mod = ctx.mod
    drop = ctx.lora_drop

    dtok = E(B * Sv, c.out_channels * p * p); ops.patchify(dout, dtok, p)
    dy2 = E(B * Sv, d); ops.gemm(dtok, P.proj_w_t, dy2, None)
    dy1 = E(B * Sv, d)
    ops.ln_modulate_bwd(dy2, ctx.y1, ctx.fm2, ctx.fr2, model.norm_out.norm.weight, (ctx.f_scale, ctx.f_scale, mod.stride(0)),
                        None, dy1, d, Sv, 0)
    dh = torch.zeros(M, d, dtype=BF16, device=dev)
    for b in range(B):
        rows = slice(b * Sv, (b + 1) * Sv)
        ops.ln_modulate_bwd(dy1[rows], ctx.h_last[b * S + St:(b + 1) * S], ctx.fm1[rows], ctx.fr1[rows],
                            model.norm_final.weight, None, None, dh[b * S + St:(b + 1) * S], d, Sv, 0)

    tg = E(M, d)
    du = E(M, c.ff_mult * d)
    dx2 = E(M, d)
    dh1 = E(M, d)
    dO = E(M, d + eo)
    dq = E(B, S, d, dt=torch.float32)
    dkh = E(M, d)
    dqkv = E(M, 3 * d)
    dx1 = E(M, d + eq)
    delta = E(B * H * S, dt=torch.float32)
    chain_ws = ops.attn_bwd_chain_workspace(B, H, S, dev)
    dh_in = E(M, d)
    for i in reversed(range(L)):
        Lw, a = P.layers[i], ctx.blocks[i]
        if ctx.recompute:
            _, a = block_forward(model, i, a.h_in, mod, ctx.dims, ctx.rope, True, ctx.scratch, drop)
        m1, m2 = _mod(mod, 2 * i, d), _mod(mod, 2 * i + 1, d)
        ops.gate_mul(dh, tg, m2.gate_txt, m2.gate_vid, m2.bs, d, S, St)
        ops.gemm(tg, Lw.w2_t, du, None, epilogue=EPI_DGELU, pre_act_in=a.u)
        ops.gemm(du, Lw.w1_t, dx2, None)
        ops.ln_modulate_bwd(dx2, a.h1, a.mean2, a.rstd2, Lw.n2g, (m2.scale_txt, m2.scale_vid, m2.bs), dh, dh1, d, S, St)
        ops.gate_mul(dh1, tg, m1.gate_txt, m1.gate_vid, m1.bs, d, S, St)
        ops.gemm(tg, Lw.w_o_t, dO, None)
        tn(tg, a.o[:, d:], r, st.b_out(st.grad, i), r, 1, st.scaling, d)
        _lora_da(st, i, "out", a.o, dO, d, drop)
        _lora_dx(st, i, "out", dO, d, drop)
        dq.zero_()
        qk3, qkv3 = a.qkh.view(B, S, 2 * d), a.qkv.view(B, S, 3 * d)
        ops.attn_bwd(qk3[:, :, :d], qk3[:, :, d:], qkv3[:, :, 2 * d:], a.o.view(B, S, d + eo)[:, :, :d],
                     dO.view(B, S, d + eo)[:, :, :d], a.lse, delta, dq, dkh.view(B, S, d),
                     dqkv.view(B, S, 3 * d)[:, :, 2 * d:], B, H, S, q_prescaled=True, chain_ws=chain_ws)
        ops.qk_layernorm_bwd(dq.view(M, d), dkh, a.qkv, a.qmean, a.qrstd, Lw.gq, Lw.gk, dqkv, H, rope=ctx.rope)
        if i > 0:
            ops.gemm(dqkv, Lw.w_qkv_t, dx1, None)
        else:
            ops.gemm(dqkv, Lw.w_qkv_t[d:], dx1[:, d:], None)
        for j in range(3):
            tn(dqkv[:, j * d:], a.x1[:, d + j * rp:], r, st.b_qkv(st.grad, i)[j * d:], r, 1, st.scaling, d)
        _lora_da(st, i, "qkv", a.x1, dx1, d, drop)
        if i > 0:
            _lora_dx(st, i, "qkv", dx1, d, drop)
            ops.ln_modulate_bwd(dx1, a.h_in, a.mean1, a.rstd1, Lw.n1g, (m1.scale_txt, m1.scale_vid, m1.bs), dh1, dh_in,
                                d, S, St)
            dh, dh_in = dh_in, dh
        ctx.blocks[i] = None
    return None


class _DiTFn(torch.autograd.Function):
    @staticmethod
    def forward(ctx, anchor, model, x, text, t, rope):
        out, saved = run_forward(model, x, text, t, save=True, rope=rope)
        ctx.model, ctx.saved = model, saved
        return out

    @staticmethod
    def backward(ctx, dout):
        if getattr(ctx.model, "fullft", None) is not None:
            from .engine_fullft import run_backward_fullft
            run_backward_fullft(ctx.model, ctx.saved, dout.contiguous(), ctx.model.fullft.on_grads_ready)
        else:
            run_backward(ctx.model, ctx.saved, dout.contiguous())
        ctx.saved = None
        return None, None, None, None, None, None


def _rope_tables(model, image_rotary_emb, Sv: int, dev):
    if image_rotary_emb is None:
        return None
    cos, sin = image_rotary_emb
    out = []
    for tb in (cos, sin):
        if tuple(tb.shape) != (Sv, model.config.attention_head_dim):
            raise ValueError(f"image_rotary_emb tables must be [{Sv}, {model.config.attention_head_dim}], got {tuple(tb.shape)}")
        out.append(tb.detach().to(device=dev, dtype=torch.float32).contiguous())
    return out[0], out[1]


def dit_apply(model, hidden_states, encoder_hidden_states, timestep, image_rotary_emb=None):
    x = hidden_states
    if x.dtype != BF16:
        raise TypeError(f"hidden_states must be bf16 (model dtype), got {x.dtype}")
    x = x.contiguous()
    text = encoder_hidden_states
    if text.dtype == torch.float32:
        tb = torch.empty(text.shape, dtype=BF16, device=text.device)
        ops.cast_f32_bf16(text.contiguous(), tb)
        text = tb
    text = text.contiguous()
    if timestep.dim() == 0:
        timestep = timestep[None].expand(x.shape[0])
    t = timestep.to(torch.int64).contiguous()
    st = model.lora
    need_grad = torch.is_grad_enabled() and ((st is not None and any(p.requires_grad for p in st.params))
                                             or getattr(model, "fullft", None) is not None)
    p = model.config.patch_size
    rope = _rope_tables(model, image_rotary_emb, x.shape[1] * (x.shape[3] // p) * (x.shape[4] // p), x.device)
    if not need_grad:
        out, _ = run_forward(model, x, text, t, save=False, rope=rope)
        return out
    anchor = torch.zeros(1, device=x.device, requires_grad=True)
    return _DiTFn.apply(anchor, model, x, text, t, rope)
```

videotuna-dev_amd/ops.py:

```python
from __future__ import annotations

import math
import os
from typing import Optional

import torch

from ._lib import check, load_library

BF16 = torch.bfloat16
EPI_BIAS, EPI_BIAS_GELU, EPI_GATED_RES, EPI_DGELU = 0, 1, 2, 3


def _stream() -> int:
    return torch.cuda.current_stream().cuda_stream


_PROFILE = {"on": False, "events": {}, "work": {}}
_PROFILED = ("attn_fwd", "attn_bwd", "conv", "conv_dw")


def profile_reset(on: bool):
    _PROFILE["on"] = on
    if on:
# ... 226 lines not shown

def _cl_check(t, nm):
    ld = t.stride(3)
    N, T, H, W, _ = t.shape
    if t.stride(2) != W * ld or t.stride(1) != H * W * ld or t.stride(0) != T * H * W * ld:
        raise ValueError(f"{nm}: positions must be uniformly strided (channels-last, only the channel axis may be a slice)")


def causal_conv3d(x, wk, bias, y, residual=None):
    _req(x, BF16, "x", 5); _req(y, BF16, "y", 5); _req(wk, BF16, "wk", 2)
    N, T, H, W, Cin = x.shape
    Cout = y.shape[4]
    if tuple(y.shape[:4]) != (N, T, H, W) or tuple(wk.shape) != (Cout, 27 * Cin) or not wk.is_contiguous():
        raise ValueError(f"shape mismatch: x {tuple(x.shape)} wk {tuple(wk.shape)} y {tuple(y.shape)}")
    _cl_check(x, "x"); _cl_check(y, "y")
    if residual is not None:
        _req(residual, BF16, "residual", 5); _cl_check(residual, "residual")
        if tuple(residual.shape) != tuple(y.shape):
            raise ValueError("residual must have the shape of y")
    check(load_library().vt_causal_conv3d_cl(x.data_ptr(), x.stride(3), wk.data_ptr(), _p(bias), _p(residual),
                                             0 if residual is None else residual.stride(3), y.data_ptr(), y.stride(3),
                                             N, T, H, W, Cin, Cout, _stream()), "vt_causal_conv3d_cl")
    return y


def pack_conv_in8_weight(w: torch.Tensor) -> torch.Tensor:
    if w.dim() != 5 or tuple(w.shape[2:]) != (3, 3, 3) or w.shape[1] > 8:
        raise ValueError(f"expected a [Cout, Cin<=8, 3, 3, 3] weight, got {tuple(w.shape)}")
    out = torch.zeros(w.shape[0], 32, 8, dtype=w.dtype, device=w.device)
    out[:, :27, :w.shape[1]] = w.permute(0, 2, 3, 4, 1).reshape(w.shape[0], 27, w.shape[1])
    return out.reshape(w.shape[0], 256)


def causal_conv3d_in8(x, wk, bias, y):
    _req(x, BF16, "x", 5); _req(y, BF16, "y", 5); _req(wk, BF16, "wk", 2)
    N, T, H, W, C8 = x.shape
    Cout = y.shape[4]
    if C8 != 8 or not x.is_contiguous() or tuple(y.shape[:4]) != (N, T, H, W) or tuple(wk.shape) != (Cout, 256) or not wk.is_contiguous():
        raise ValueError(f"shape mismatch: x {tuple(x.shape)} wk {tuple(wk.shape)} y {tuple(y.shape)}")
    _cl_check(y, "y")
    check(load_library().vt_causal_conv3d_in8_cl(x.data_ptr(), wk.data_ptr(), _p(bias), y.data_ptr(), y.stride(3), N, T, H, W, Cout,
                                                 _stream()), "vt_causal_conv3d_in8_cl")
    return y


def downsample_conv2d(x, wk, bias, y):
    _req(x, BF16, "x", 5); _req(y, BF16, "y", 5); _req(wk, BF16, "wk", 2)
    N, T, H, W, Cin = x.shape
    Cout = y.shape[4]
    if tuple(y.shape[:4]) != (N, T, H // 2, W // 2) or tuple(wk.shape) != (Cout, 9 * Cin) or not wk.is_contiguous():
        raise ValueError(f"shape mismatch: x {tuple(x.shape)} wk {tuple(wk.shape)} y {tuple(y.shape)}")
    _cl_check(x, "x"); _cl_check(y, "y")
    check(load_library().vt_downsample_conv2d_cl(x.data_ptr(), x.stride(3), wk.data_ptr(), _p(bias), y.data_ptr(), y.stride(3),
                                                 N, T, H, W, Cin, Cout, _stream()), "vt_downsample_conv2d_cl")
    return y


def temporal_pool_frames(T: int, keep_first: bool) -> int:
    return 1 + (T - 1) // 2 if keep_first else T // 2


def temporal_pool(x, y, keep_first: bool = True):
    _req(x, BF16, "x", 5); _req(y, BF16, "y", 5)
    N, T, H, W, C = x.shape
    To = temporal_pool_frames(T, keep_first)
    if tuple(y.shape) != (N, To, H, W, C) or To < 1:
        raise ValueError(f"y must be {(N, To, H, W, C)}, got {tuple(y.shape)}")
    _cl_check(x, "x"); _cl_check(y, "y")
    check(load_library().vt_temporal_pool_cl(x.data_ptr(), x.stride(3), y.data_ptr(), y.stride(3), N, T, H * W, C, int(keep_first),
                                             _stream()), "vt_temporal_pool_cl")
    return y


def rmsnorm(x, w, y, eps: float = 1e-6):
    _req(x, BF16, "x", 2); _req(y, BF16, "y", 2); _req(w, BF16, "w", 1)
    check(load_library().vt_rmsnorm_bf16(x.data_ptr(), x.stride(0), w.data_ptr(), y.data_ptr(), y.stride(0), x.shape[0], x.shape[1],
                                         eps, _stream()), "vt_rmsnorm_bf16")


def gated_gelu(u, y):
    _req(u, BF16, "u", 2); _req(y, BF16, "y", 2)
    check(load_library().vt_gated_gelu_bf16(u.data_ptr(), u.stride(0), y.data_ptr(), y.stride(0), u.shape[0], y.shape[1], _stream()),
          "vt_gated_gelu_bf16")


def attn_bwd_chain_workspace(B: int, H: int, S: int, device) -> Optional[torch.Tensor]:
    if _SIDE_STREAMS["n"] > 0 or _CHAIN_STATE["disabled"]:
        return None
    n = int(load_library().vt_attn_bwd_chain_ws_bytes(B, H, S))
    if n <= 0:
        return None
    key = str(device)
    ws = _CHAIN_WS.get(key)
    if ws is None or ws.numel() < n:
        old = ws
        ws = _CHAIN_WS[key] = torch.empty(n, dtype=torch.uint8, device=device)
        ws[:256].zero_()
        if old is not None:
            ws[64:256].copy_(old[64:256])
    return ws


_CHAIN_WS = {}
_SIDE_STREAMS = {"n": 0}
_CHAIN_STATE = {"disabled": False, "redone": 0, "verify": __import__("os").environ.get("VT355_CHAIN_VERIFY", "launch")}


def attn_bwd_chain_redone() -> int:
    return _CHAIN_STATE["redone"]


def declare_side_stream(active: bool):
    _SIDE_STREAMS["n"] = max(0, _SIDE_STREAMS["n"] + (1 if active else -1))


def chain_guard(device) -> Optional[torch.Tensor]:
    ws = _CHAIN_WS.get(str(device))
    return None if ws is None else ws[64:68].view(torch.int32)


def attn_bwd_chain_errors() -> int:
    return sum(int(ws[64:68].view(torch.int32).item()) for ws in _CHAIN_WS.values())


def attn_bwd_chain_errors_clear():
    for ws in _CHAIN_WS.values():
        ws[64:256].zero_()


def conv_set_tile(mode: int = 0):
    check(load_library().vt_conv_set_tile(mode), "vt_conv_set_tile")


def gemm_set_tile(mode: int = 0):
    check(load_library().vt_gemm_set_tile(mode), "vt_gemm_set_tile")


def gemm_kernel(M: int, N: int, K: int) -> int:
    k = load_library().vt_gemm_bf16_kernel(M, N, K)
    if k < 0:
        check(k, "vt_gemm_bf16_kernel")
    return k


def attn_bwd_set_chain(chain_len: int = 0, slots: int = 0):
    check(load_library().vt_attn_bwd_set_chain(chain_len, slots), "vt_attn_bwd_set_chain")


def attn_bwd_chain_error(chain_ws: torch.Tensor) -> int:
    return int(chain_ws[32:36].view(torch.int32).item())


def attn_bwd(q, k, v, o, do, lse2, delta_ws, dq_f32, dk, dv, B: int, H: int, S: int, scale: Optional[float] = None,
             q_prescaled: bool = False, chain_ws: Optional[torch.Tensor] = None, _entry=None):
    scale = 1.0 / math.sqrt(64) if scale is None else scale
    for n, t in (("q", q), ("k", k), ("v", v), ("o", o), ("do", do), ("dk", dk), ("dv", dv)):
        _req(t, BF16, n, 3)
    _req(dq_f32, torch.float32, "dq_f32", 3)
    lib = load_library()

    def launch(ws, fn=None):
        check((fn or lib.vt_attn_bwd_hd64)(q.data_ptr(), k.data_ptr(), v.data_ptr(), o.data_ptr(), do.data_ptr(),
                               lse2.data_ptr(), delta_ws.data_ptr(), dq_f32.data_ptr(), dk.data_ptr(), dv.data_ptr(),
                               B, H, S,
                               q.stride(1), k.stride(1), v.stride(1), o.stride(1), do.stride(1),
                               dq_f32.stride(1), dk.stride(1), dv.stride(1),
                               q.stride(0), k.stride(0), v.stride(0), o.stride(0), do.stride(0),
                               dq_f32.stride(0), dk.stride(0), dv.stride(0), scale, int(q_prescaled),
                               None if ws is None else ws.data_ptr(), 0 if ws is None else ws.numel(),
                               _stream()),
          "vt_attn_bwd_hd64")
    with _timed("attn_bwd"):
        launch(chain_ws, _entry)
    if chain_ws is not None and _CHAIN_STATE["verify"] == "launch" and attn_bwd_chain_error(chain_ws) != 0:
        import warnings
        _CHAIN_STATE["disabled"] = True
        _CHAIN_STATE["redone"] += 1
        warnings.warn("vt_attn_bwd_hd64: a dQ hand-off wait timed out (the persistent workgroups were not all resident: another stream or a "
                      "profiler shared the CUs); the launch was redone with plain atomics and the hand-off chains are switched off for the rest "
                      "of this process (VT_BWD_CHAIN=1 avoids them from the start; ops.declare_side_stream(True) announces a concurrent stream)")
        dq_f32.zero_()
        launch(None)
        chain_ws[32:36].zero_()
        chain_ws[64:68].zero_()


def ln_modulate_fwd(x, y, gamma, beta, mod, mean, rstd, D: int, S: int, St: int, eps: float):
    _req(x, BF16, "x", 2); _req(y, BF16, "y", 2)
    m = (None, None, None, None, 0) if mod is None else mod
    lib = load_library()
    with _timed_hbm("ln_modulate_fwd", x.shape[0], 4.0 * x.shape[0] * D):
        check(lib.vt_ln_modulate_fwd(x.data_ptr(), x.stride(0), y.data_ptr(), y.stride(0), _p(gamma), _p(beta),
                                     _p(m[0]), _p(m[1]), _p(m[2]), _p(m[3]), m[4], _p(mean), _p(rstd),
                                     x.shape[0], D, S, St, eps, _stream()), "vt_ln_modulate_fwd")


def ln_modulate_bwd(dy, x, mean, rstd, gamma, scales, dres, dx, D: int, S: int, St: int):
    _req(dy, BF16, "dy", 2); _req(x, BF16, "x", 2); _req(dx, BF16, "dx", 2)
    sc = (None, None, 0) if scales is None else scales
    lib = load_library()
    with _timed_hbm("ln_modulate_bwd", x.shape[0], (6.0 if dres is None else 8.0) * x.shape[0] * D):
        check(lib.vt_ln_modulate_bwd(dy.data_ptr(), dy.stride(0), x.data_ptr(), x.stride(0), mean.data_ptr(), rstd.data_ptr(),
                                     _p(gamma), _p(sc[0]), _p(sc[1]), sc[2], _p(dres), 0 if dres is None else dres.stride(0),
                                     dx.data_ptr(), dx.stride(0), x.shape[0], D, S, St, _stream()), "vt_ln_modulate_bwd")


def qk_layernorm_fwd(qkv, out, gq, bq, gk, bk, mean, rstd, H: int, eps: float, q_scale: float = 1.0, rope=None):
    _req(qkv, BF16, "qkv", 2); _req(out, BF16, "out", 2)
    lib = load_library()
    rc, rsn, S, St = _rope_args(rope, qkv.shape[0])
    with _timed_hbm("qk_layernorm_fwd", qkv.shape[0], 8.0 * qkv.shape[0] * H * 64):
        check(lib.vt_qk_layernorm_fwd(qkv.data_ptr(), qkv.stride(0), out.data_ptr(), out.stride(0), gq.data_ptr(), bq.data_ptr(),
                                      gk.data_ptr(), bk.data_ptr(), mean.data_ptr(), rstd.data_ptr(), qkv.shape[0], H, eps,
                                      q_scale, rc, rsn, S, St, _stream()), "vt_qk_layernorm_fwd")


def qk_layernorm_bwd(dq_hat_f32, dk_hat, qkv, mean, rstd, gq, gk, dqkv, H: int, rope=None):
    _req(dq_hat_f32, torch.float32, "dq_hat", 2); _req(dk_hat, BF16, "dk_hat", 2)
    lib = load_library()
    rc, rsn, S, St = _rope_args(rope, qkv.shape[0])
    with _timed_hbm("qk_layernorm_bwd", qkv.shape[0], 14.0 * qkv.shape[0] * H * 64):
        check(lib.vt_qk_layernorm_bwd(dq_hat_f32.data_ptr(), dq_hat_f32.stride(0), dk_hat.data_ptr(), dk_hat.stride(0),
                                      qkv.data_ptr(), qkv.stride(0), mean.data_ptr(), rstd.data_ptr(), gq.data_ptr(), gk.data_ptr(),
                                      dqkv.data_ptr(), dqkv.stride(0), qkv.shape[0], H, rc, rsn, S, St, _stream()),
              "vt_qk_layernorm_bwd")


def gate_mul(x, y, g_txt, g_vid, bstride: int, D: int, S: int, St: int):
    _req(x, BF16, "x", 2); _req(y, BF16, "y", 2)
    lib = load_library()
    check(lib.vt_gate_mul(x.data_ptr(), x.stride(0), y.data_ptr(), y.stride(0), g_txt.data_ptr(), g_vid.data_ptr(), bstride,
                          x.shape[0], D, S, St, _stream()), "vt_gate_mul")


def silu(x, y):
    _req(x, BF16, "x"); _req(y, BF16, "y")
    check(load_library().vt_silu_bf16(x.data_ptr(), y.data_ptr(), x.numel(), _stream()), "vt_silu_bf16")


def cast_f32_bf16(x, y):
    _req(x, torch.float32, "x"); _req(y, BF16, "y")
    check(load_library().vt_cast_f32_bf16(x.data_ptr(), y.data_ptr(), x.numel(), _stream()), "vt_cast_f32_bf16")


def timestep_embedding(t, out, flip: bool = True, freq_shift: float = 0.0):
    _req(t, torch.int64, "t", 1); _req(out, BF16, "out", 2)
    check(load_library().vt_timestep_embedding(t.data_ptr(), out.data_ptr(), out.shape[0], out.shape[1], int(flip),
                                               freq_shift, _stream()), "vt_timestep_embedding")


def patchify(img, tok, P: int):
    _req(img, BF16, "img", 5); _req(tok, BF16, "tok", 2)
    B, F, C, H, W = img.shape
    check(load_library().vt_patchify(img.data_ptr(), tok.data_ptr(), B, F, C, H, W, P, tok.stride(0), _stream()), "vt_patchify")


def unpatchify(tok, img, P: int):
    _req(img, BF16, "img", 5); _req(tok, BF16, "tok", 2)
    B, F, C, H, W = img.shape
    check(load_library().vt_unpatchify(tok.data_ptr(), img.data_ptr(), B, F, C, H, W, P, tok.stride(0), _stream()),
          "vt_unpatchify")


def add_noise(x0, noise, sa, sb, noisy):
    _req(x0, torch.float32, "x0"); _req(noise, torch.float32, "noise"); _req(noisy, BF16, "noisy")
    B = x0.shape[0]
    check(load_library().vt_add_noise(x0.data_ptr(), noise.data_ptr(), sa.data_ptr(), sb.data_ptr(), noisy.data_ptr(),
                                      x0.numel() // B, B, _stream()), "vt_add_noise")


def diffusion_loss(vpred, noisy, x0, sa, sb, w, loss, partials, dvpred, grad_scale: float = 1.0):
    _req(vpred, BF16, "vpred"); _req(noisy, BF16, "noisy"); _req(x0, torch.float32, "x0")
    B = x0.shape[0]
    check(load_library().vt_diffusion_loss(vpred.data_ptr(), noisy.data_ptr(), x0.data_ptr(), sa.data_ptr(), sb.data_ptr(),
                                           w.data_ptr(), loss.data_ptr(), partials.data_ptr(), _p(dvpred),
                                           x0.numel() // B, B, grad_scale, _stream()), "vt_diffusion_loss")


def diffusion_loss_bwd(vpred, noisy, x0, sa, sb, w, grad_out, dvpred):
    _req(grad_out, torch.float32, "grad_out")
    B = x0.shape[0]
    check(load_library().vt_diffusion_loss_bwd(vpred.data_ptr(), noisy.data_ptr(), x0.data_ptr(), sa.data_ptr(), sb.data_ptr(),
                                               w.data_ptr(), grad_out.data_ptr(), dvpred.data_ptr(), x0.numel() // B, B,
                                               _stream()), "vt_diffusion_loss_bwd")


def adamw(p, g, m, v, p_bf16, lr, beta1, beta2, eps, wd, step: int, grad_scale: float = 1.0, guard: Optional[torch.Tensor] = None,
          clip_coef: Optional[torch.Tensor] = None, clip_value: float = 0.0):
    for n, t in (("p", p), ("g", g), ("m", m), ("v", v)):
        _req(t, torch.float32, n)
    if guard is not None:
        _req(guard, torch.int32, "guard")
    with _timed_hbm("adamw", p.numel(), (28.0 + (2.0 if p_bf16 is not None else 0.0)) * p.numel()):
        if clip_coef is None and not clip_value > 0.0:
            check(load_library().vt_adamw(p.data_ptr(), g.data_ptr(), m.data_ptr(), v.data_ptr(), _p(p_bf16), p.numel(),
                                          lr, beta1, beta2, eps, wd, step, grad_scale, _p(guard), _stream()), "vt_adamw")
        else:
            if clip_coef is not None:
                _req(clip_coef, torch.float32, "clip_coef")
            check(load_library().vt_adamw_clip(p.data_ptr(), g.data_ptr(), m.data_ptr(), v.data_ptr(), _p(p_bf16), p.numel(),
                                               lr, beta1, beta2, eps, wd, step, grad_scale, _p(guard), _p(clip_coef),
                                               float(clip_value), _stream()), "vt_adamw_clip")


def grad_sqnorm_partials() -> int:
    return int(load_library().vt_grad_sqnorm_partials())


def grad_sqnorm(g, partials, slot: int = 0):
    _req(g, torch.float32, "g"); _req(partials, torch.float32, "partials")
    if partials.numel() < (slot + 1) * grad_sqnorm_partials():
        raise ValueError("partials holds fewer than slot + 1 slots")
    check(load_library().vt_grad_sqnorm(g.data_ptr(), g.numel(), partials.data_ptr(), slot, _stream()), "vt_grad_sqnorm")


def clip_finalize(partials, nslots: int, grad_scale: float, max_norm: float, record):
    _req(partials, torch.float32, "partials"); _req(record, torch.float32, "record")
    if partials.numel() < nslots * grad_sqnorm_partials() or record.numel() < 2:
        raise ValueError("partials / record too small")
    check(load_library().vt_clip_finalize(partials.data_ptr(), nslots, float(grad_scale), float(max_norm), record.data_ptr(),
                                          _stream()), "vt_clip_finalize")


def lora_down(x, a, R: int, t_out, K: int, zero_cols: int = 48):
    _req(x, BF16, "x", 2); _req(a, BF16, "a", 2); _req(t_out, BF16, "t", 2)
    check(load_library().vt_lora_down(x.data_ptr(), x.stride(0), a.data_ptr(), a.stride(0), R, t_out.data_ptr(),
                                      t_out.stride(0), x.shape[0], K, zero_cols, _stream()), "vt_lora_down")


_SKINNY_WS = {}


def _skinny_ws(lib, big, P: int, use_workspace: bool):
    if not use_workspace:
        return None
    need = lib.vt_skinny_tn_workspace_bytes(P) // 4
    key = big.device
    if key not in _SKINNY_WS or _SKINNY_WS[key].numel() < need:
        _SKINNY_WS[key] = torch.empty(need, dtype=torch.float32, device=big.device)
    return _SKINNY_WS[key]


def skinny_tn(big, small, R: int, out, osp: int, osr: int, alpha: float, P: int, use_workspace: bool = False):
    _req(big, BF16, "big", 2); _req(small, BF16, "small", 2); _req(out, torch.float32, "out")
    lib = load_library()
    ws = _skinny_ws(lib, big, P, use_workspace)
    check(lib.vt_skinny_tn(big.data_ptr(), big.stride(0), small.data_ptr(), small.stride(0), R, out.data_ptr(),
                           osp, osr, alpha, big.shape[0], P, _p(ws), _stream()), "vt_skinny_tn")


def lora_up_add(dx, dt, a, R: int, K: int):
    _req(dx, BF16, "dx", 2); _req(dt, BF16, "dt", 2); _req(a, BF16, "a", 2)
    check(load_library().vt_lora_up_add(dx.data_ptr(), dx.stride(0), dt.data_ptr(), dt.stride(0), a.data_ptr(), a.stride(0),
                                        R, dx.shape[0], K, _stream()), "vt_lora_up_add")


def lora_pack_b(bcat_f32, wext, ldw: int, n_adapters: int, d_out: int, r: int, scale: float):
# ... 670 lines not shown
```

Measured before the change: 2.823 samples/s.

## Fuse LoRA input-grad up-projection into layernorm backward and attention delta kernels

Adds a delta kernel that folds the out-projection LoRA dx update (dT·A) into dO in place while computing the attention backward row-sum delta, and a variant of the attention backward entry that skips its own delta pass. It also extends the modulated layernorm backward kernel to apply the qkv LoRA dx update before normalization and to write the gated gradient for the next layer, which removes separate _lora_dx and gate_mul launches. The aim is fewer full-tensor HBM passes over M×d activations per layer in the backward. The cost is staging the LoRA A matrix in LDS and capping the grid size, and the fused path is used only for narrow, non-dropout configurations.

Result: no change. 2.826 samples/s (median of 3 runs) (+0.1%).

```diff
diff --git a/include/vt355.h b/include/vt355.h
--- a/include/vt355.h
+++ b/include/vt355.h
@@ -87,6 +87,16 @@
                      float softmax_scale, int q_prescaled, void* chain_ws, long long chain_ws_bytes, void* stream);
 long long vt_attn_bwd_chain_ws_bytes(int B, int H, int S);
 int vt_attn_bwd_set_chain(int chain_len, int slots);
+int vt_attn_bwd_hd64_delta_in(const void* q, const void* k, const void* v, const void* o, const void* dout,
+                              const float* lse2, float* delta_ws, float* dq_f32, void* dk, void* dv,
+                              int B, int H, int S,
+                              long long q_rs, long long k_rs, long long v_rs, long long o_rs, long long do_rs,
+                              long long dq_rs, long long dk_rs, long long dv_rs,
+                              long long q_bs, long long k_bs, long long v_bs, long long o_bs, long long do_bs,
+                              long long dq_bs, long long dk_bs, long long dv_bs,
+                              float softmax_scale, int q_prescaled, void* chain_ws, long long chain_ws_bytes, void* stream);
+int vt_attn_bwd_delta_lora(const void* o, void* dout, const void* dT, int ldt, const void* A, int lda, int R, float* delta_ws,
+                           int B, int H, int S, long long o_rs, long long do_rs, long long o_bs, long long do_bs, void* stream);
 
 int vt_ln_modulate_fwd(const void* x, int ldx, void* y, int ldy, const void* gamma, const void* beta,
                        const float* shift_txt, const float* scale_txt, const float* shift_vid,
@@ -96,6 +106,12 @@
                        const void* gamma, const float* scale_txt, const float* scale_vid, int mod_bstride,
                        const void* dres, int lddres, void* dx, int lddx,
                        int M, int D, int S, int St, void* stream);
+int vt_ln_modulate_bwd_lora(const void* dy, int lddy, const void* x, int ldx, const float* mean, const float* rstd,
+                            const void* gamma, const float* scale_txt, const float* scale_vid, int mod_bstride,
+                            const void* dres, int lddres, void* dx, int lddx,
+                            const void* dT, int ldt, const void* A, int lda, int R,
+                            void* gy, int ldgy, const float* gate_txt, const float* gate_vid, int gate_bstride,
+                            int M, int D, int S, int St, void* stream);
 
 int vt_qk_layernorm_fwd(const void* qkv, int ld, void* out, int ldo, const void* gq, const void* bq,
                         const void* gk, const void* bk, float* mean, float* rstd,
diff --git a/videotuna-dev_amd/_lib.py b/videotuna-dev_amd/_lib.py
--- a/videotuna-dev_amd/_lib.py
+++ b/videotuna-dev_amd/_lib.py
@@ -46,10 +46,15 @@
     "vt_gated_gelu_bf16": [_vp, _ll, _vp, _ll, _ll, _i, _vp],
     "vt_attn_bwd_hd64": [_vp, _vp, _vp, _vp, _vp, _fp, _fp, _fp, _vp, _vp, _i, _i, _i,
                          _ll, _ll, _ll, _ll, _ll, _ll, _ll, _ll, _ll, _ll, _ll, _ll, _ll, _ll, _ll, _ll, _f, _i, _vp, _ll, _vp],
+    "vt_attn_bwd_hd64_delta_in": [_vp, _vp, _vp, _vp, _vp, _fp, _fp, _fp, _vp, _vp, _i, _i, _i,
+                                  _ll, _ll, _ll, _ll, _ll, _ll, _ll, _ll, _ll, _ll, _ll, _ll, _ll, _ll, _ll, _ll, _f, _i, _vp, _ll, _vp],
+    "vt_attn_bwd_delta_lora": [_vp, _vp, _vp, _i, _vp, _i, _i, _fp, _i, _i, _i, _ll, _ll, _ll, _ll, _vp],
     "vt_attn_bwd_chain_ws_bytes": [_i, _i, _i],
     "vt_attn_bwd_set_chain": [_i, _i],
     "vt_ln_modulate_fwd": [_vp, _i, _vp, _i, _vp, _vp, _fp, _fp, _fp, _fp, _i, _fp, _fp, _i, _i, _i, _i, _f, _vp],
     "vt_ln_modulate_bwd": [_vp, _i, _vp, _i, _fp, _fp, _vp, _fp, _fp, _i, _vp, _i, _vp, _i, _i, _i, _i, _i, _vp],
+    "vt_ln_modulate_bwd_lora": [_vp, _i, _vp, _i, _fp, _fp, _vp, _fp, _fp, _i, _vp, _i, _vp, _i, _vp, _i, _vp, _i, _i,
+                                _vp, _i, _fp, _fp, _i, _i, _i, _i, _i, _vp],
     "vt_qk_layernorm_fwd": [_vp, _i, _vp, _i, _vp, _vp, _vp, _vp, _fp, _fp, _ll, _i, _f, _f, _fp, _fp, _i, _i, _vp],
     "vt_qk_layernorm_bwd": [_fp, _i, _vp, _i, _vp, _i, _fp, _fp, _vp, _vp, _vp, _i, _ll, _i, _fp, _fp, _i, _i, _vp],
     "vt_gate_mul": [_vp, _i, _vp, _i, _fp, _fp, _i, _ll, _i, _i, _i, _vp],
diff --git a/videotuna-dev_amd/csrc/attn_bwd.hip b/videotuna-dev_amd/csrc/attn_bwd.hip
--- a/videotuna-dev_amd/csrc/attn_bwd.hip
+++ b/videotuna-dev_amd/csrc/attn_bwd.hip
@@ -81,6 +81,9 @@
 #define BWD_BODY VT_CAT(attn_bwd_body, VT_SUFFIX)
 #define DELTA_KERNEL VT_CAT(attn_bwd_delta_kernel, VT_SUFFIX)
 #define BWD_ENTRY VT_CAT(vt_attn_bwd_hd64, VT_SUFFIX)
+#define DELTA_LORA_KERNEL VT_CAT(attn_bwd_delta_lora_kernel, VT_SUFFIX)
+#define DELTA_LORA_ENTRY VT_CAT(vt_attn_bwd_delta_lora, VT_SUFFIX)
+#define BWD_DELTA_IN_ENTRY VT_CAT(vt_attn_bwd_hd64_delta_in, VT_SUFFIX)
 
 struct AttnBwdParams {
     const bf16_t* q;
@@ -1717,6 +1720,54 @@
     }
 }
 
+__global__ __launch_bounds__(256) void DELTA_LORA_KERNEL(const bf16_t* o, bf16_t* dout, const bf16_t* dT, int ldt, const bf16_t* A, int lda,
+                                                         int R, float* delta, int B, int H, int S, long long o_rs, long long do_rs,
+                                                         long long o_bs, long long do_bs) {
+    extern __shared__ __attribute__((aligned(16))) unsigned char delta_lora_smem[];
+    bf16_t* As = (bf16_t*)delta_lora_smem;
+    const int K = H * 64, nchunks = H * 8;
+    for (int i = threadIdx.x; i < R * nchunks; i += 256) {
+        const int r = i / nchunks, c = i - r * nchunks;
+        *(u32x4*)(As + (size_t)r * K + c * 8) = *(const u32x4*)(A + (size_t)r * lda + c * 8);
+    }
+    __syncthreads();
+    const long long total = (long long)B * S * H;
+    for (long long base = (long long)blockIdx.x * 256; base < total * 8; base += (long long)gridDim.x * 256) {
+        const long long gid = base + threadIdx.x;
+        const long long row = gid >> 3;
+        const int sub = (int)(gid & 7);
+        float acc = 0.f;
+        long long bs = 0; int hh = 0;
+        if (row < total) {
+            hh = (int)(row % H);
+            bs = row / H;
+            const int s = (int)(bs % S);
+            const int b = (int)(bs / S);
+            bf16_t* dp = dout + (size_t)b * do_bs + (size_t)s * do_rs + hh * 64 + sub * 8;
+            u32x4 a = *(const u32x4*)(o + (size_t)b * o_bs + (size_t)s * o_rs + hh * 64 + sub * 8);
+            float v[8];
+            unpack8(*(const u32x4*)dp, v);
+            for (int r = 0; r < R; ++r)
+                lora_up_fma8(v, bf2f(dT[(size_t)bs * ldt + r]), *(const u32x4*)(As + (size_t)r * K + hh * 64 + sub * 8));
+            u32x4 c = pack8(v);
+            *(u32x4*)dp = c;
+            float fa[8], fc[8];
+            unpack8(a, fa);
+            unpack8(c, fc);
+#pragma unroll
+            for (int i = 0; i < 8; ++i) acc += fa[i] * fc[i];
+        }
+        acc += __shfl_xor(acc, 1, 64);
+        acc += __shfl_xor(acc, 2, 64);
+        acc += __shfl_xor(acc, 4, 64);
+        if (row < total && sub == 0) {
+            const int s = (int)(bs % S);
+            const int b = (int)(bs / S);
+            delta[((size_t)b * H + hh) * S + s] = acc;
+        }
+    }
+}
+
 static long long bwd_chain_xcc_off(long long slots) { return 256 + slots * 64; }
 static long long bwd_chain_tiles_off(long long slots) { return (256 + slots * 68 + 4095) & ~4095LL; }
 static long long bwd_chain_ws_bytes(long long slots) { return bwd_chain_tiles_off(slots) + slots * (long long)(CH_R * 16384); }
@@ -1744,7 +1795,7 @@
     return VT_OK;
 }
 
-extern "C" int BWD_ENTRY(const void* q, const void* k, const void* v, const void* o, const void* dout,
+static int bwd_launch(bool own_delta, const void* q, const void* k, const void* v, const void* o, const void* dout,
                                 const float* lse2, float* delta_ws, float* dq_f32, void* dk, void* dv,
                                 int B, int H, int S,
                                 long long q_rs, long long k_rs, long long v_rs, long long o_rs, long long do_rs,
@@ -1763,7 +1814,7 @@
     if ((long long)S * q_rs * 2 >= lim || (long long)S * k_rs * 2 >= lim || (long long)S * v_rs * 2 >= lim ||
         (long long)S * do_rs * 2 >= lim) return VT_ERR_BAD_SHAPE;
     hipStream_t st = (hipStream_t)stream;
-    {
+    if (own_delta) {
         const long long total = (long long)B * S * H * 8;
         const int blocks = (int)((total + 255) / 256);
         hipLaunchKernelGGL(DELTA_KERNEL, dim3(blocks), dim3(256), 0, st, (const bf16_t*)o, (const bf16_t*)dout,
@@ -1803,6 +1854,37 @@
     return hipGetLastError() == hipSuccess ? VT_OK : VT_ERR_LAUNCH;
 }
 
+#define BWD_ARGS_DECL const void* q, const void* k, const void* v, const void* o, const void* dout, \
+                      const float* lse2, float* delta_ws, float* dq_f32, void* dk, void* dv, int B, int H, int S, \
+                      long long q_rs, long long k_rs, long long v_rs, long long o_rs, long long do_rs, \
+                      long long dq_rs, long long dk_rs, long long dv_rs, \
+                      long long q_bs, long long k_bs, long long v_bs, long long o_bs, long long do_bs, \
+                      long long dq_bs, long long dk_bs, long long dv_bs, \
+                      float softmax_scale, int q_prescaled, void* chain_ws, long long chain_ws_bytes, void* stream
+#define BWD_ARGS q, k, v, o, dout, lse2, delta_ws, dq_f32, dk, dv, B, H, S, q_rs, k_rs, v_rs, o_rs, do_rs, dq_rs, dk_rs, dv_rs, \
+                 q_bs, k_bs, v_bs, o_bs, do_bs, dq_bs, dk_bs, dv_bs, softmax_scale, q_prescaled, chain_ws, chain_ws_bytes, stream
+extern "C" int BWD_ENTRY(BWD_ARGS_DECL) { return bwd_launch(true, BWD_ARGS); }
+extern "C" int BWD_DELTA_IN_ENTRY(BWD_ARGS_DECL) { return bwd_launch(false, BWD_ARGS); }
+#undef BWD_ARGS
+#undef BWD_ARGS_DECL
+
+#define DELTA_LORA_MAX_WGS 2048
+extern "C" int DELTA_LORA_ENTRY(const void* o, void* dout, const void* dT, int ldt, const void* A, int lda, int R, float* delta_ws,
+                                int B, int H, int S, long long o_rs, long long do_rs, long long o_bs, long long do_bs, void* stream) {
+    if (B <= 0 || H <= 0 || S <= 0 || R <= 0 || R > 16 || (lda % 8) || lda < H * 64) return VT_ERR_BAD_SHAPE;
+    if ((o_rs % 8) || (do_rs % 8) || (o_bs % 8) || (do_bs % 8)) return VT_ERR_BAD_SHAPE;
+    if (dT == nullptr || A == nullptr || delta_ws == nullptr) return VT_ERR_BAD_SHAPE;
+    if ((((uintptr_t)o) | ((uintptr_t)dout) | ((uintptr_t)A)) & 15) return VT_ERR_BAD_ALIGN;
+    const size_t lds = (size_t)R * H * 64 * sizeof(bf16_t);
+    if (lds > 65536) return VT_ERR_UNSUPPORTED;
+    const long long total = (long long)B * S * H * 8;
+    const long long blocks = (total + 255) / 256;
+    hipLaunchKernelGGL(DELTA_LORA_KERNEL, dim3((unsigned)(blocks < DELTA_LORA_MAX_WGS ? blocks : DELTA_LORA_MAX_WGS)), dim3(256), lds,
+                       (hipStream_t)stream, (const bf16_t*)o, (bf16_t*)dout, (const bf16_t*)dT, ldt, (const bf16_t*)A, lda, R, delta_ws,
+                       B, H, S, o_rs, do_rs, o_bs, do_bs);
+    return hipGetLastError() == hipSuccess ? VT_OK : VT_ERR_LAUNCH;
+}
+
 #if VT_STAMP
 extern "C" int VT_CAT(vt_attn_bwd_stamps, VT_SUFFIX)(unsigned* host_out) {
     return hipMemcpyFromSymbol(host_out, HIP_SYMBOL(VT_CAT(vt_bwd_stamps, VT_SUFFIX)), 256 * sizeof(unsigned)) == hipSuccess ? VT_OK : VT_ERR_LAUNCH;
diff --git a/videotuna-dev_amd/csrc/common.h b/videotuna-dev_amd/csrc/common.h
--- a/videotuna-dev_amd/csrc/common.h
+++ b/videotuna-dev_amd/csrc/common.h
@@ -46,6 +46,13 @@
 #pragma unroll
     for (int i = 0; i < 4; ++i) v[i] = pack2(f[2 * i], f[2 * i + 1]);
     return v;
+}
+
+__device__ __forceinline__ void lora_up_fma8(float* acc, float t, const u32x4& araw) {
+    float a[8];
+    unpack8(araw, a);
+#pragma unroll
+    for (int q = 0; q < 8; ++q) acc[q] = __builtin_fmaf(t, a[q], acc[q]);
 }
 
 __device__ __forceinline__ float wave_sum(float v) {
diff --git a/videotuna-dev_amd/csrc/lora.hip b/videotuna-dev_amd/csrc/lora.hip
--- a/videotuna-dev_amd/csrc/lora.hip
+++ b/videotuna-dev_amd/csrc/lora.hip
@@ -255,10 +255,7 @@
             float(&acc)[8] = DROP ? s : v;
             for (int ri = j * r; ri < (j + 1) * r; ++ri) {
                 const float t = bf2f(dT[(size_t)m * ldt + ri]);
-                float a[8];
-                unpack8(*(const u32x4*)(A + (size_t)ri * lda + c * 8), a);
-#pragma unroll
-                for (int q = 0; q < 8; ++q) acc[q] += t * a[q];
+                lora_up_fma8(acc, t, *(const u32x4*)(A + (size_t)ri * lda + c * 8));
             }
             if constexpr (DROP) {
                 unsigned rnd[8];
diff --git a/videotuna-dev_amd/csrc/norm.hip b/videotuna-dev_amd/csrc/norm.hip
--- a/videotuna-dev_amd/csrc/norm.hip
+++ b/videotuna-dev_amd/csrc/norm.hip
@@ -123,70 +123,149 @@
     int M, D, S, St;
 };
 
-template <int NCH>
-__global__ __launch_bounds__(256) void ln_modulate_bwd_kernel(LnBwdParams p) {
+struct LnBwdLora {
+    const bf16_t* dT; int ldt; const bf16_t* A; int lda; int R;
+    bf16_t* gy; int ldgy; const float* gate_txt; const float* gate_vid; int gate_bstride;
+};
+
+__device__ __forceinline__ LnBwdLora ln_bwd_lora_arg() { return LnBwdLora{}; }
+__device__ __forceinline__ LnBwdLora ln_bwd_lora_arg(const LnBwdLora& f) { return f; }
+
+template <int NCH, typename... F>
+__global__ __launch_bounds__(256) void ln_modulate_bwd_kernel(LnBwdParams p, F... fused) {
+    constexpr bool FUSED = sizeof...(F) > 0;
+    const LnBwdLora f = ln_bwd_lora_arg(fused...);
     const int lane = threadIdx.x & 63;
-    const int m = blockIdx.x * 4 + (threadIdx.x >> 6);
+    extern __shared__ __attribute__((aligned(16))) unsigned char ln_lora_smem[];
+    const bf16_t* As = (const bf16_t*)ln_lora_smem;
+    if constexpr (FUSED) {
+        if (f.dT != nullptr) {
+            const int nchunks = p.D >> 3;
+            for (int i = threadIdx.x; i < f.R * nchunks; i += 256) {
+                const int r = i / nchunks, c = i - r * nchunks;
+                *(u32x4*)(ln_lora_smem + ((size_t)r * p.D + c * 8) * sizeof(bf16_t)) = *(const u32x4*)(f.A + (size_t)r * f.lda + c * 8);
+            }
+            __syncthreads();
+        }
+    }
+    int m = blockIdx.x * 4 + (threadIdx.x >> 6);
     if (m >= p.M) return;
-    const int nchunks = p.D >> 3;
-    const float mean = p.mean[m], rstd = p.rstd[m];
-    const float* scp = nullptr;
-    if (p.scale_vid != nullptr) {
-        const int b = m / p.S;
-        const int s = m - b * p.S;
-        scp = (s < p.St ? p.scale_txt : p.scale_vid) + (size_t)b * p.mod_bstride;
-    }
-    float gv[NCH][8], xh[NCH][8];
-    float s1 = 0.f, s2 = 0.f;
-#pragma unroll
-    for (int i = 0; i < NCH; ++i) {
-        const int c = lane + 64 * i;
-        if (c < nchunks) {
-            float dyv[8], xv[8];
-            unpack8(*(const u32x4*)(p.dy + (size_t)m * p.lddy + c * 8), dyv);
-            unpack8(*(const u32x4*)(p.x + (size_t)m * p.ldx + c * 8), xv);
-            float ga[8];
-            if (p.gamma != nullptr) unpack8(*(const u32x4*)(p.gamma + c * 8), ga);
-            float sc8[8];
-            if (scp != nullptr) {
-                f32x4 a = *(const f32x4*)(scp + c * 8), bq = *(const f32x4*)(scp + c * 8 + 4);
-#pragma unroll
-                for (int j = 0; j < 4; ++j) { sc8[j] = 1.f + a[j]; sc8[j + 4] = 1.f + bq[j]; }
-            }
-#pragma unroll
-            for (int j = 0; j < 8; ++j) {
-                float gg = dyv[j];
-                if (scp != nullptr) gg *= sc8[j];
-                if (p.gamma != nullptr) gg *= ga[j];
-                float xhat = (xv[j] - mean) * rstd;
-                gv[i][j] = gg;
-                xh[i][j] = xhat;
-                s1 += gg;
-                s2 += gg * xhat;
-            }
-        } else {
-#pragma unroll
-            for (int j = 0; j < 8; ++j) { gv[i][j] = 0.f; xh[i][j] = 0.f; }
-        }
-    }
-    const float invD = 1.f / (float)p.D;
-    const float m1 = wave_sum(s1) * invD, m2 = wave_sum(s2) * invD;
-#pragma unroll
-    for (int i = 0; i < NCH; ++i) {
-        const int c = lane + 64 * i;
-        if (c < nchunks) {
-            float o[8];
-#pragma unroll
-            for (int j = 0; j < 8; ++j) o[j] = rstd * (gv[i][j] - m1 - xh[i][j] * m2);
-            if (p.dres != nullptr) {
-                float dr[8];
-                unpack8(*(const u32x4*)(p.dres + (size_t)m * p.lddres + c * 8), dr);
-#pragma unroll
-                for (int j = 0; j < 8; ++j) o[j] += dr[j];
-            }
-            *(u32x4*)(p.dx + (size_t)m * p.lddx + c * 8) = pack8(o);
-        }
-    }
+    do {
+        const int nchunks = p.D >> 3;
+        const float mean = p.mean[m], rstd = p.rstd[m];
+        const float* scp = nullptr;
+        if (p.scale_vid != nullptr) {
+            const int b = m / p.S;
+            const int s = m - b * p.S;
+            scp = (s < p.St ? p.scale_txt : p.scale_vid) + (size_t)b * p.mod_bstride;
+        }
+        float gv[NCH][8], xh[NCH][8];
+        if constexpr (FUSED) {
+            if (f.dT != nullptr) {
+#pragma unroll
+                for (int i = 0; i < NCH; ++i) {
+                    const int c = lane + 64 * i;
+                    if (c < nchunks) unpack8(*(const u32x4*)(p.dy + (size_t)m * p.lddy + c * 8), gv[i]);
+                }
+                for (int r = 0; r < f.R; ++r) {
+                    const float t = bf2f(f.dT[(size_t)m * f.ldt + r]);
+#pragma unroll
+                    for (int i = 0; i < NCH; ++i) {
+                        const int c = lane + 64 * i;
+                        if (c < nchunks) lora_up_fma8(gv[i], t, *(const u32x4*)(As + (size_t)r * p.D + c * 8));
+                    }
+                }
+#pragma unroll
+                for (int i = 0; i < NCH; ++i) {
+                    if (lane + 64 * i < nchunks) {
+                        const u32x4 rounded = pack8(gv[i]);
+                        unpack8(rounded, gv[i]);
+                    }
+                }
+            }
+        }
+        float s1 = 0.f, s2 = 0.f;
+#pragma unroll
+        for (int i = 0; i < NCH; ++i) {
+            const int c = lane + 64 * i;
+            if (c < nchunks) {
+                float dyv[8], xv[8];
+                if constexpr (FUSED) {
+                    if (f.dT != nullptr) {
+#pragma unroll
+                        for (int j = 0; j < 8; ++j) dyv[j] = gv[i][j];
+                    } else {
+                        unpack8(*(const u32x4*)(p.dy + (size_t)m * p.lddy + c * 8), dyv);
+                    }
+                } else {
+                    unpack8(*(const u32x4*)(p.dy + (size_t)m * p.lddy + c * 8), dyv);
+                }
+                unpack8(*(const u32x4*)(p.x + (size_t)m * p.ldx + c * 8), xv);
+                float ga[8];
+                if (p.gamma != nullptr) unpack8(*(const u32x4*)(p.gamma + c * 8), ga);
+                float sc8[8];
+                if (scp != nullptr) {
+                    f32x4 a = *(const f32x4*)(scp + c * 8), bq = *(const f32x4*)(scp + c * 8 + 4);
+#pragma unroll
+                    for (int j = 0; j < 4; ++j) { sc8[j] = 1.f + a[j]; sc8[j + 4] = 1.f + bq[j]; }
+                }
+#pragma unroll
+                for (int j = 0; j < 8; ++j) {
+                    float gg = dyv[j];
+                    if (scp != nullptr) gg *= sc8[j];
+                    if (p.gamma != nullptr) gg *= ga[j];
+                    float xhat = (xv[j] - mean) * rstd;
+                    gv[i][j] = gg;
+                    xh[i][j] = xhat;
+                    s1 += gg;
+                    s2 += gg * xhat;
+                }
+            } else {
+#pragma unroll
+                for (int j = 0; j < 8; ++j) { gv[i][j] = 0.f; xh[i][j] = 0.f; }
+            }
+        }
+        const float invD = 1.f / (float)p.D;
+        const float m1 = wave_sum(s1) * invD, m2 = wave_sum(s2) * invD;
+        const float* gate = nullptr;
+        if constexpr (FUSED) {
+            if (f.gy != nullptr) {
+                const int b = m / p.S;
+                const int s = m - b * p.S;
+                gate = (s < p.St ? f.gate_txt : f.gate_vid) + (size_t)b * f.gate_bstride;
+            }
+        }
+#pragma unroll
+        for (int i = 0; i < NCH; ++i) {
+            const int c = lane + 64 * i;
+            if (c < nchunks) {
+                float o[8];
+#pragma unroll
+                for (int j = 0; j < 8; ++j) o[j] = rstd * (gv[i][j] - m1 - xh[i][j] * m2);
+                if (p.dres != nullptr) {
+                    float dr[8];
+                    unpack8(*(const u32x4*)(p.dres + (size_t)m * p.lddres + c * 8), dr);
+#pragma unroll
+                    for (int j = 0; j < 8; ++j) o[j] += dr[j];
+                }
+                if constexpr (!FUSED) {
+                    *(u32x4*)(p.dx + (size_t)m * p.lddx + c * 8) = pack8(o);
+                } else {
+                    const u32x4 packed = pack8(o);
+                    *(u32x4*)(p.dx + (size_t)m * p.lddx + c * 8) = packed;
+                    if (gate != nullptr) {
+                        float v[8];
+                        unpack8(packed, v);
+                        f32x4 a = *(const f32x4*)(gate + c * 8), bq = *(const f32x4*)(gate + c * 8 + 4);
+#pragma unroll
+                        for (int j = 0; j < 4; ++j) { v[j] *= a[j]; v[j + 4] *= bq[j]; }
+                        *(u32x4*)(f.gy + (size_t)m * f.ldgy + c * 8) = pack8(v);
+                    }
+                }
+            }
+        }
+        m += gridDim.x * 4;
+    } while (FUSED && m < p.M);
 }
 
 static int nch_for(int D) { return ((D >> 3) + 63) / 64; }
@@ -251,6 +330,45 @@
     if (nch <= 1) hipLaunchKernelGGL(ln_modulate_bwd_kernel<1>, grid, block, 0, st, p);
     else if (nch <= 4) hipLaunchKernelGGL(ln_modulate_bwd_kernel<4>, grid, block, 0, st, p);
     else hipLaunchKernelGGL(ln_modulate_bwd_kernel<8>, grid, block, 0, st, p);
+    return hipGetLastError() == hipSuccess ? VT_OK : VT_ERR_LAUNCH;
+}
+
+#define LN_LORA_MAX_LDS 65536
+#define LN_LORA_MAX_WGS 768
+extern "C" int vt_ln_modulate_bwd_lora(const void* dy, int lddy, const void* x, int ldx, const float* mean, const float* rstd,
+                                       const void* gamma, const float* scale_txt, const float* scale_vid, int mod_bstride,
+                                       const void* dres, int lddres, void* dx, int lddx,
+                                       const void* dT, int ldt, const void* A, int lda, int R,
+                                       void* gy, int ldgy, const float* gate_txt, const float* gate_vid, int gate_bstride,
+                                       int M, int D, int S, int St, void* stream) {
+    if (M <= 0 || M > 0x7fffffff - 4 * LN_LORA_MAX_WGS || D <= 0 || (D % 8) || D > 4096 || (ldx % 8) || (lddy % 8) || (lddx % 8))
+        return VT_ERR_BAD_SHAPE;
+    if (dres != nullptr && (lddres % 8)) return VT_ERR_BAD_SHAPE;
+    if (scale_vid != nullptr && (scale_txt == nullptr || (mod_bstride % 4))) return VT_ERR_BAD_SHAPE;
+    if ((((uintptr_t)x) | ((uintptr_t)dy) | ((uintptr_t)dx) | ((uintptr_t)dres)) & 15) return VT_ERR_BAD_ALIGN;
+    if ((dT == nullptr) != (A == nullptr)) return VT_ERR_BAD_SHAPE;
+    size_t lds = 0;
+    if (dT != nullptr) {
+        if (R <= 0 || R > 16 || (lda % 8) || lda < D) return VT_ERR_BAD_SHAPE;
+        if (((uintptr_t)A) & 15) return VT_ERR_BAD_ALIGN;
+        lds = (size_t)R * D * sizeof(bf16_t);
+        if (lds > LN_LORA_MAX_LDS) return VT_ERR_UNSUPPORTED;
+    }
+    if (gy != nullptr) {
+        if (gate_txt == nullptr || gate_vid == nullptr || (gate_bstride % 4) || (ldgy % 8) || S <= 0) return VT_ERR_BAD_SHAPE;
+        if ((((uintptr_t)gy) | ((uintptr_t)gate_txt) | ((uintptr_t)gate_vid)) & 15) return VT_ERR_BAD_ALIGN;
+    }
+    LnBwdParams p{(const bf16_t*)dy, lddy, (const bf16_t*)x, ldx, mean, rstd, (const bf16_t*)gamma,
+                  scale_txt, scale_vid, mod_bstride, (const bf16_t*)dres, lddres, (bf16_t*)dx, lddx,
+                  M, D, S > 0 ? S : 1, St};
+    LnBwdLora f{(const bf16_t*)dT, ldt, (const bf16_t*)A, lda, R, (bf16_t*)gy, ldgy, gate_txt, gate_vid, gate_bstride};
+    const int groups = (M + 3) / 4;
+    dim3 grid(groups < LN_LORA_MAX_WGS ? groups : LN_LORA_MAX_WGS), block(256);
+    hipStream_t st = (hipStream_t)stream;
+    const int nch = nch_for(D);
+    if (nch <= 1) hipLaunchKernelGGL((ln_modulate_bwd_kernel<1, LnBwdLora>), grid, block, lds, st, p, f);
+    else if (nch <= 4) hipLaunchKernelGGL((ln_modulate_bwd_kernel<4, LnBwdLora>), grid, block, lds, st, p, f);
+    else hipLaunchKernelGGL((ln_modulate_bwd_kernel<8, LnBwdLora>), grid, block, lds, st, p, f);
     return hipGetLastError() == hipSuccess ? VT_OK : VT_ERR_LAUNCH;
 }
 
diff --git a/videotuna-dev_amd/engine.py b/videotuna-dev_amd/engine.py
--- a/videotuna-dev_amd/engine.py
+++ b/videotuna-dev_amd/engine.py
@@ -1,5 +1,6 @@
 from __future__ import annotations
 
+import os
 from types import SimpleNamespace
 from typing import List, Optional
 
@@ -391,25 +392,36 @@
     delta = E(B * H * S, dt=torch.float32)
     chain_ws = ops.attn_bwd_chain_workspace(B, H, S, dev)
     dh_in = E(M, d)
+    fused = (not st.wide and drop is None and 3 * r <= 16 and 3 * r * d * 2 <= ops.LN_BWD_LORA_MAX_A_BYTES
+             and os.environ.get("VT355_FUSED_LORA_BWD") != "0")
+    tg_ready = False
     for i in reversed(range(L)):
         Lw, a = P.layers[i], ctx.blocks[i]
         if ctx.recompute:
             _, a = block_forward(model, i, a.h_in, mod, ctx.dims, ctx.rope, True, ctx.scratch, drop)
         m1, m2 = _mod(mod, 2 * i, d), _mod(mod, 2 * i + 1, d)
-        ops.gate_mul(dh, tg, m2.gate_txt, m2.gate_vid, m2.bs, d, S, St)
+        if not tg_ready:
+            ops.gate_mul(dh, tg, m2.gate_txt, m2.gate_vid, m2.bs, d, S, St)
         ops.gemm(tg, Lw.w2_t, du, None, epilogue=EPI_DGELU, pre_act_in=a.u)
         ops.gemm(du, Lw.w1_t, dx2, None)
-        ops.ln_modulate_bwd(dx2, a.h1, a.mean2, a.rstd2, Lw.n2g, (m2.scale_txt, m2.scale_vid, m2.bs), dh, dh1, d, S, St)
-        ops.gate_mul(dh1, tg, m1.gate_txt, m1.gate_vid, m1.bs, d, S, St)
+        if fused:
+            ops.ln_modulate_bwd_lora(dx2, a.h1, a.mean2, a.rstd2, Lw.n2g, (m2.scale_txt, m2.scale_vid, m2.bs), dh, dh1, d, S, St,
+                                     gated=(tg, m1.gate_txt, m1.gate_vid, m1.bs))
+        else:
+            ops.ln_modulate_bwd(dx2, a.h1, a.mean2, a.rstd2, Lw.n2g, (m2.scale_txt, m2.scale_vid, m2.bs), dh, dh1, d, S, St)
+            ops.gate_mul(dh1, tg, m1.gate_txt, m1.gate_vid, m1.bs, d, S, St)
         ops.gemm(tg, Lw.w_o_t, dO, None)
         tn(tg, a.o[:, d:], r, st.b_out(st.grad, i), r, 1, st.scaling, d)
         _lora_da(st, i, "out", a.o, dO, d, drop)
-        _lora_dx(st, i, "out", dO, d, drop)
+        o3, dO3 = a.o.view(B, S, d + eo)[:, :, :d], dO.view(B, S, d + eo)[:, :, :d]
+        if fused:
+            ops.attn_bwd_delta_lora(o3, dO3, dO[:, d:], st.a_out(st.flat_bf16, i), r, delta, B, H, S)
+        else:
+            _lora_dx(st, i, "out", dO, d, drop)
         dq.zero_()
         qk3, qkv3 = a.qkh.view(B, S, 2 * d), a.qkv.view(B, S, 3 * d)
-        ops.attn_bwd(qk3[:, :, :d], qk3[:, :, d:], qkv3[:, :, 2 * d:], a.o.view(B, S, d + eo)[:, :, :d],
-                     dO.view(B, S, d + eo)[:, :, :d], a.lse, delta, dq, dkh.view(B, S, d),
-                     dqkv.view(B, S, 3 * d)[:, :, 2 * d:], B, H, S, q_prescaled=True, chain_ws=chain_ws)
+        ops.attn_bwd(qk3[:, :, :d], qk3[:, :, d:], qkv3[:, :, 2 * d:], o3, dO3, a.lse, delta, dq, dkh.view(B, S, d),
+                     dqkv.view(B, S, 3 * d)[:, :, 2 * d:], B, H, S, q_prescaled=True, chain_ws=chain_ws, delta_in=fused)
         ops.qk_layernorm_bwd(dq.view(M, d), dkh, a.qkv, a.qmean, a.qrstd, Lw.gq, Lw.gk, dqkv, H, rope=ctx.rope)
         if i > 0:
             ops.gemm(dqkv, Lw.w_qkv_t, dx1, None)
@@ -418,7 +430,13 @@
         for j in range(3):
             tn(dqkv[:, j * d:], a.x1[:, d + j * rp:], r, st.b_qkv(st.grad, i)[j * d:], r, 1, st.scaling, d)
         _lora_da(st, i, "qkv", a.x1, dx1, d, drop)
-        if i > 0:
+        if i > 0 and fused:
+            mp = _mod(mod, 2 * i - 1, d)
+            ops.ln_modulate_bwd_lora(dx1, a.h_in, a.mean1, a.rstd1, Lw.n1g, (m1.scale_txt, m1.scale_vid, m1.bs), dh1, dh_in, d, S, St,
+                                     lora=(dx1[:, d:], st.a_qkv(st.flat_bf16, i), 3 * r), gated=(tg, mp.gate_txt, mp.gate_vid, mp.bs))
+            dh, dh_in = dh_in, dh
+            tg_ready = True
+        elif i > 0:
             _lora_dx(st, i, "qkv", dx1, d, drop)
             ops.ln_modulate_bwd(dx1, a.h_in, a.mean1, a.rstd1, Lw.n1g, (m1.scale_txt, m1.scale_vid, m1.bs), dh1, dh_in,
                                 d, S, St)
diff --git a/videotuna-dev_amd/ops.py b/videotuna-dev_amd/ops.py
--- a/videotuna-dev_amd/ops.py
+++ b/videotuna-dev_amd/ops.py
@@ -402,7 +402,7 @@
 
 
 def attn_bwd(q, k, v, o, do, lse2, delta_ws, dq_f32, dk, dv, B: int, H: int, S: int, scale: Optional[float] = None,
-             q_prescaled: bool = False, chain_ws: Optional[torch.Tensor] = None, _entry=None):
+             q_prescaled: bool = False, chain_ws: Optional[torch.Tensor] = None, _entry=None, delta_in: bool = False):
     scale = 1.0 / math.sqrt(64) if scale is None else scale
     for n, t in (("q", q), ("k", k), ("v", v), ("o", o), ("do", do), ("dk", dk), ("dv", dv)):
         _req(t, BF16, n, 3)
@@ -410,7 +410,7 @@
     lib = load_library()
 
     def launch(ws, fn=None):
-        check((fn or lib.vt_attn_bwd_hd64)(q.data_ptr(), k.data_ptr(), v.data_ptr(), o.data_ptr(), do.data_ptr(),
+        check((fn or (lib.vt_attn_bwd_hd64_delta_in if delta_in else lib.vt_attn_bwd_hd64))(q.data_ptr(), k.data_ptr(), v.data_ptr(), o.data_ptr(), do.data_ptr(),
                                lse2.data_ptr(), delta_ws.data_ptr(), dq_f32.data_ptr(), dk.data_ptr(), dv.data_ptr(),
                                B, H, S,
                                q.stride(1), k.stride(1), v.stride(1), o.stride(1), do.stride(1),
@@ -435,6 +435,14 @@
         chain_ws[64:68].zero_()
 
 
+def attn_bwd_delta_lora(o, do, dt, a, R: int, delta_ws, B: int, H: int, S: int):
+    _req(o, BF16, "o", 3); _req(do, BF16, "do", 3); _req(dt, BF16, "dt", 2); _req(a, BF16, "a", 2)
+    _req(delta_ws, torch.float32, "delta_ws")
+    check(load_library().vt_attn_bwd_delta_lora(o.data_ptr(), do.data_ptr(), dt.data_ptr(), dt.stride(0), a.data_ptr(), a.stride(0), R,
+                                                delta_ws.data_ptr(), B, H, S, o.stride(1), do.stride(1), o.stride(0), do.stride(0),
+                                                _stream()), "vt_attn_bwd_delta_lora")
+
+
 def ln_modulate_fwd(x, y, gamma, beta, mod, mean, rstd, D: int, S: int, St: int, eps: float):
     _req(x, BF16, "x", 2); _req(y, BF16, "y", 2)
     m = (None, None, None, None, 0) if mod is None else mod
@@ -453,6 +461,29 @@
         check(lib.vt_ln_modulate_bwd(dy.data_ptr(), dy.stride(0), x.data_ptr(), x.stride(0), mean.data_ptr(), rstd.data_ptr(),
                                      _p(gamma), _p(sc[0]), _p(sc[1]), sc[2], _p(dres), 0 if dres is None else dres.stride(0),
                                      dx.data_ptr(), dx.stride(0), x.shape[0], D, S, St, _stream()), "vt_ln_modulate_bwd")
+
+
+LN_BWD_LORA_MAX_A_BYTES = 65536
+
+
+def ln_modulate_bwd_lora(dy, x, mean, rstd, gamma, scales, dres, dx, D: int, S: int, St: int, lora=None, gated=None):
+    _req(dy, BF16, "dy", 2); _req(x, BF16, "x", 2); _req(dx, BF16, "dx", 2)
+    sc = (None, None, 0) if scales is None else scales
+    dt, a, R = (None, None, 0) if lora is None else lora
+    gy, g_txt, g_vid, gbs = (None, None, None, 0) if gated is None else gated
+    if dt is not None:
+        _req(dt, BF16, "dt", 2); _req(a, BF16, "a", 2)
+    if gy is not None:
+        _req(gy, BF16, "gy", 2)
+    lib = load_library()
+    nbytes = (6.0 + (0.0 if dres is None else 2.0) + (0.0 if gy is None else 2.0)) * x.shape[0] * D
+    with _timed_hbm("ln_modulate_bwd", x.shape[0], nbytes):
+        check(lib.vt_ln_modulate_bwd_lora(dy.data_ptr(), dy.stride(0), x.data_ptr(), x.stride(0), mean.data_ptr(), rstd.data_ptr(),
+                                          _p(gamma), _p(sc[0]), _p(sc[1]), sc[2], _p(dres), 0 if dres is None else dres.stride(0),
+                                          dx.data_ptr(), dx.stride(0),
+                                          _p(dt), 0 if dt is None else dt.stride(0), _p(a), 0 if a is None else a.stride(0), R,
+                                          _p(gy), 0 if gy is None else gy.stride(0), _p(g_txt), _p(g_vid), gbs,
+                                          x.shape[0], D, S, St, _stream()), "vt_ln_modulate_bwd_lora")
 
 
 def qk_layernorm_fwd(qkv, out, gq, bq, gk, bk, mean, rstd, H: int, eps: float, q_scale: float = 1.0, rope=None):
```
